# widdowquinn/pyani

Hardware: AMD Instinct MI355X
Metric: genome-pairs/sec (ordered pairs) + wall-clock for the N x N ANIm grid: nucmer --mum + delta-filter -1 + parse_delta equivalent per ordered pair, genomes resident in HBM; vs the CPU path on this box's host cores (higher is better)
Workload: dtype u32 packed DP words (score << 17 | state << 15 | errors), i64 lengths, f64 identity

## Files before the change

### include/pyani_gpu.h

```cpp
#ifndef PYANI_GPU_H
#define PYANI_GPU_H

#include <stdint.h>

#ifdef __cplusplus
extern "C" {
#endif

#define PG_OK 0
#define PG_E_ARG (-1)
#define PG_E_NODEVICE (-2)
#define PG_E_HIP (-3)
#define PG_E_IO (-4)
#define PG_E_NOMEM (-5)
#define PG_E_KEYSET (-6)
#define PG_E_EMPTY (-7)
#define PG_E_RNA (-8)
#define PG_E_CAPACITY (-9)
#define PG_E_INTERNAL (-10)

typedef struct pg_ctx pg_ctx;

const char* pg_version(void);
int pg_create(pg_ctx** out, int device);
void pg_destroy(pg_ctx* ctx);
const char* pg_last_error(const pg_ctx* ctx);
int pg_sync(pg_ctx* ctx);

int pg_add_genome(pg_ctx* ctx, const uint8_t* seq, const uint64_t* rec_off, uint32_t n_rec, int32_t* genome_id_out);
int pg_add_fasta(pg_ctx* ctx, const char* path, int32_t* genome_id_out, uint64_t* total_len_out, uint32_t* n_rec_out);
int pg_add_fasta_batch(pg_ctx* ctx, const char* const* paths, uint32_t n, uint32_t threads, int32_t* genome_ids_out,
                       uint64_t* total_len_out, uint32_t* n_rec_out);
int pg_genome_count(const pg_ctx* ctx);
int pg_genome_length(const pg_ctx* ctx, int32_t genome_id, uint64_t* total_len_out, uint32_t* n_rec_out);
int pg_clear_genomes(pg_ctx* ctx);
int pg_upload(pg_ctx* ctx);
int pg_tetra_algorithmic_bytes(const pg_ctx* ctx, const int32_t* genome_ids, uint32_t n, uint64_t* bytes_out,
                               uint64_t* bases_out);

int pg_tetra_counts(pg_ctx* ctx, const int32_t* genome_ids, uint32_t n, uint64_t* c2, uint64_t* c3, uint64_t* c4);

int pg_tetra_zscores(pg_ctx* ctx, const uint64_t* c2, const uint64_t* c3, const uint64_t* c4, uint32_t n, double* z,
                     uint8_t* present);

int pg_tetra_corr(pg_ctx* ctx, const double* z, const uint8_t* present, uint32_t n, double* out);

int pg_tetra_matrix(pg_ctx* ctx, const int32_t* genome_ids, uint32_t n, double* z_out, uint8_t* present_out,
                    double* corr_out);
int pg_tetra_matrix_enqueue(pg_ctx* ctx, const int32_t* genome_ids, uint32_t n, int fetch_z);
int pg_tetra_matrix_fetch(pg_ctx* ctx, uint32_t n, double* z_out, uint8_t* present_out, double* corr_out);

int pg_tetra_zscores_dev(pg_ctx* ctx, const int32_t* genome_ids, uint32_t n, double* d_z, uint8_t* d_present);
int pg_tetra_corr_rows_dev(pg_ctx* ctx, const double* d_z, const uint8_t* d_present, uint32_t n, uint32_t row0,
                           uint32_t nrows, double* d_out);

typedef struct {
  int64_t ref_aln_len, qry_aln_len, sim_errors, n_alignments;
  double identity;
  int32_t status;
  int32_t reserved;
} pg_anim_result;
#define PG_ANIM_NO_ALIGNMENT 1
int pg_anim_pairs(pg_ctx* ctx, const int32_t* ref_ids, const int32_t* qry_ids, uint64_t n_pairs, int maxmatch,
                  int filter_1to1, pg_anim_result* out);
int pg_anim_pairs_enqueue(pg_ctx* ctx, const int32_t* ref_ids, const int32_t* qry_ids, uint64_t n_pairs, int maxmatch,
                          int filter_1to1, uint64_t* ticket);
int pg_anim_pairs_fetch(pg_ctx* ctx, uint64_t ticket, pg_anim_result* out, uint64_t n_pairs);

#define PG_EXTENDER_NUCMER 0
int pg_anim_set_extender(pg_ctx* ctx, int extender);
int pg_anim_set_workers(pg_ctx* ctx, int workers);

int pg_anim_counters(pg_ctx* ctx, uint64_t* out, int reset);

int pg_anim_set_batch_budget(pg_ctx* ctx, uint32_t max_pairs, uint64_t max_matches);

typedef struct {
  int32_t ref_rec, qry_rec;
  int32_t rs, re, qs, qe;
  int32_t errors;
  int32_t kept;
} pg_anim_alignment;
int pg_anim_pair_alignments(pg_ctx* ctx, int32_t ref_id, int32_t qry_id, pg_anim_alignment* out, uint32_t cap, uint32_t* n_out);

int pg_anim_alignments_batch(pg_ctx* ctx, const int32_t* ref_ids, const int32_t* qry_ids, uint64_t n_pairs, int maxmatch, int with_indels,
                             uint64_t* aln_offsets, uint64_t* n_indels);
int pg_anim_alignments_read(pg_ctx* ctx, pg_anim_alignment* out, uint64_t* indel_offsets, int64_t* indels);

int pg_anim_reduce(pg_ctx* ctx, uint32_t n_pairs, const uint64_t* offsets, const int32_t* rseq, const int32_t* qseq,
                   const int32_t* rs, const int32_t* re, const int32_t* qs, const int32_t* qe, const int32_t* errors,
                   int apply_filter, pg_anim_result* out);

int pg_anib_reduce(pg_ctx* ctx, uint32_t n_pairs, const uint64_t* offsets, const uint32_t* n_frags, const int32_t* frag,
                   const int32_t* length, const int32_t* mismatch, const int32_t* gaps, const int32_t* qlen, const double* pident,
                   int64_t* aln_length_out, int64_t* sim_errors_out, double* pid_out);

typedef struct {
  int64_t aln_length, sim_errors;
  double pid;
  int32_t n_frags, n_kept;
  int32_t status, reserved;
} pg_anib_result;
int pg_anib_pairs(pg_ctx* ctx, const int32_t* qry_ids, const int32_t* sbj_ids, uint64_t n_pairs, uint32_t fragsize, pg_anib_result* out);
typedef struct {
  int32_t frag, length, mismatch, gaps, nident, qlen, qstart, qend, sstart, send, srec, score;
} pg_anib_row;
int pg_anib_pair_rows(pg_ctx* ctx, int32_t qry_id, int32_t sbj_id, uint32_t fragsize, pg_anib_row* out, uint32_t cap, uint32_t* n_out);

typedef struct {
  double ani;
  int32_t matches;
  int32_t fragments;
  int32_t status;
  int32_t reserved;
} pg_sketch_result;
#define PG_SKETCH_NO_RESULT 1
int pg_sketch_pairs(pg_ctx* ctx, const int32_t* qry_ids, const int32_t* ref_ids, uint64_t n_pairs, int32_t frag_len, int32_t scale,
                    double min_fraction, pg_sketch_result* out);

int pg_profile_enable(pg_ctx* ctx, int on);
int pg_profile_config(pg_ctx* ctx, uint32_t kernel_mask, uint32_t every_n);
int pg_profile_reset(pg_ctx* ctx);
#define PG_K_TETRA_COUNT 0
#define PG_K_TETRA_FINALIZE 1
#define PG_K_TETRA_STATS 2
#define PG_K_TETRA_PAIRS 3
#define PG_K_ANIM_SEED 4
#define PG_K_ANIM_HIT 5
#define PG_K_ANIM_CLUSTER 6
#define PG_K_ANIM_GAPS 7
#define PG_K_ANIM_EXTLANE 8
#define PG_K_ANIM_EXTEND 9
#define PG_K_ANIM_FINISH 10
#define PG_K_ANIB_BUCKET 11
#define PG_K_ANIB_FRAG 12
#define PG_K_ANIM_FWD 13
#define PG_K_ANIM_BWD 14
#define PG_K_SKETCH_PAIRS 15
#define PG_K__COUNT 16
int pg_profile_get(pg_ctx* ctx, int which, double* total_ms_out, uint64_t* launches_out);
const char* pg_kernel_name(int which);

#ifdef __cplusplus
}
#endif
#endif
```

### pyani_amd/_lib.py

```python
import ctypes
import os
from pathlib import Path



def configure_runtime(hw_queues: int = 2) -> bool:
    if not 1 <= int(hw_queues) <= 2:
        raise ValueError(f"hw_queues must be 1 or 2, not {hw_queues}")
    os.environ.setdefault("GPU_MAX_HW_QUEUES", str(int(hw_queues)))
    return _lib is None

LIB_PATH = Path(__file__).resolve().parent / "libpyani_gpu.so"

PG_OK, PG_E_ARG, PG_E_NODEVICE, PG_E_HIP, PG_E_IO, PG_E_NOMEM, PG_E_KEYSET, PG_E_EMPTY, PG_E_RNA = 0, -1, -2, -3, -4, -5, -6, -7, -8
PG_E_CAPACITY, PG_ANIM_NO_ALIGNMENT = -9, 1
K_TETRA_COUNT, K_TETRA_FINALIZE, K_TETRA_STATS, K_TETRA_PAIRS = 0, 1, 2, 3
(K_ANIM_SEED, K_ANIM_HIT, K_ANIM_CLUSTER, K_ANIM_GAPS, K_ANIM_EXTLANE, K_ANIM_EXTEND, K_ANIM_FINISH) = 4, 5, 6, 7, 8, 9, 10
K_ANIB_BUCKET, K_ANIB_FRAG = 11, 12
K_ANIM_FWD, K_ANIM_BWD = 13, 14
K_SKETCH_PAIRS = 15
K_COUNT = 16
PG_SKETCH_NO_RESULT = 1

_vp, _i32, _u32, _u64, _int = ctypes.c_void_p, ctypes.c_int32, ctypes.c_uint32, ctypes.c_uint64, ctypes.c_int
_P = ctypes.POINTER
SIGNATURES = {
    "pg_version": (ctypes.c_char_p, []),
    "pg_create": (_int, [_P(_vp), _int]),
    "pg_destroy": (None, [_vp]),
    "pg_last_error": (ctypes.c_char_p, [_vp]),
    "pg_sync": (_int, [_vp]),
    "pg_add_genome": (_int, [_vp, _vp, _vp, _u32, _P(_i32)]),
    "pg_add_fasta": (_int, [_vp, ctypes.c_char_p, _P(_i32), _P(_u64), _P(_u32)]),
    "pg_add_fasta_batch": (_int, [_vp, _vp, _u32, _u32, _vp, _vp, _vp]),
    "pg_genome_count": (_int, [_vp]),
    "pg_genome_length": (_int, [_vp, _i32, _P(_u64), _P(_u32)]),
    "pg_clear_genomes": (_int, [_vp]),
    "pg_upload": (_int, [_vp]),
    "pg_tetra_algorithmic_bytes": (_int, [_vp, _vp, _u32, _P(_u64), _P(_u64)]),
    "pg_tetra_counts": (_int, [_vp, _vp, _u32, _vp, _vp, _vp]),
    "pg_tetra_zscores": (_int, [_vp, _vp, _vp, _vp, _u32, _vp, _vp]),
    "pg_tetra_corr": (_int, [_vp, _vp, _vp, _u32, _vp]),
    "pg_tetra_matrix": (_int, [_vp, _vp, _u32, _vp, _vp, _vp]),
    "pg_tetra_matrix_enqueue": (_int, [_vp, _vp, _u32, _int]),
    "pg_tetra_matrix_fetch": (_int, [_vp, _u32, _vp, _vp, _vp]),
    "pg_tetra_zscores_dev": (_int, [_vp, _vp, _u32, _vp, _vp]),
    "pg_tetra_corr_rows_dev": (_int, [_vp, _vp, _vp, _u32, _u32, _u32, _vp]),
    "pg_anim_pairs": (_int, [_vp, _vp, _vp, _u64, _int, _int, _vp]),
    "pg_anim_pairs_enqueue": (_int, [_vp, _vp, _vp, _u64, _int, _int, _vp]),
    "pg_anim_pairs_fetch": (_int, [_vp, _u64, _vp, _u64]),
    "pg_anim_reduce": (_int, [_vp, _u32, _vp, _vp, _vp, _vp, _vp, _vp, _vp, _vp, _int, _vp]),
    "pg_anim_set_batch_budget": (_int, [_vp, _u32, ctypes.c_uint64]),
    "pg_anim_set_workers": (_int, [_vp, _int]),
    "pg_anim_set_extender": (_int, [_vp, _int]),
    "pg_anim_counters": (_int, [_vp, _vp, _int]),
    "pg_anim_pair_alignments": (_int, [_vp, _i32, _i32, _vp, _u32, _P(_u32)]),
    "pg_anim_alignments_batch": (_int, [_vp, _vp, _vp, _u64, _int, _int, _vp, _P(_u64)]),
    "pg_anim_alignments_read": (_int, [_vp, _vp, _vp, _vp]),
    "pg_anib_reduce": (_int, [_vp, _u32, _vp, _vp, _vp, _vp, _vp, _vp, _vp, _vp, _vp, _vp, _vp]),
    "pg_anib_pairs": (_int, [_vp, _vp, _vp, _u64, _u32, _vp]),
    "pg_anib_pair_rows": (_int, [_vp, _i32, _i32, _u32, _vp, _u32, _P(_u32)]),
    "pg_sketch_pairs": (_int, [_vp, _vp, _vp, _u64, _i32, _i32, ctypes.c_double, _vp]),
    "pg_profile_enable": (_int, [_vp, _int]),
    "pg_profile_config": (_int, [_vp, _u32, _u32]),
    "pg_profile_reset": (_int, [_vp]),
    "pg_profile_get": (_int, [_vp, _int, _P(ctypes.c_double), _P(_u64)]),
    "pg_kernel_name": (ctypes.c_char_p, [_int]),
}

_lib = None


class PyaniGpuError(RuntimeError):

    def __init__(self, code, msg):
        super().__init__(f"libpyani_gpu error {code}: {msg}")
        self.code = code


def load():
    global _lib
    if _lib is None:
        if not LIB_PATH.exists():
            raise ImportError(f"{LIB_PATH} not built — run `python -m pyani_amd.build` (needs hipcc); "
                              "pyani_amd has no CPU fallback")
        lib = ctypes.CDLL(str(LIB_PATH))
        for name, (res, args) in SIGNATURES.items():
            fn = getattr(lib, name)
            fn.restype, fn.argtypes = res, args
        _lib = lib
    return _lib
```

### pyani_amd/csrc/pg_anim.hip

```cpp
#include <tuple>
#include "pg_internal.h"
#include "pg_anim_core.h"
#include "pg_nucmer_core.h"
#include "pg_nucmer_diag.h"
#include "pg_anib_core.h"
#include "pg_anim_trace.h"

using namespace pga;

namespace {

constexpr unsigned long long SLOT_EMPTY = ~0ull;
constexpr int FRAG_SEED_MIN = 16;

struct RefDesc {
  const uint32_t* codes;
  const uint32_t* mask;
  int32_t len;
  const int32_t* rec_start;
  int32_t n_rec;
};

struct UnitDesc {
  const uint32_t* codes;
// ... 70 lines not shown
  int32_t *nch = nullptr, *status = nullptr;
  pg_anim_result* out = nullptr;
  Match *mem = nullptr, *cm = nullptr;
  int32_t *iscratch = nullptr, *order = nullptr;
  Chain* chains = nullptr;
  FinishScratch S{};
  uint2* wl_d = nullptr;
  Match* seedbuf = nullptr;
  size_t seed_cap = 0;
  uint32_t* seed_total = nullptr;
  Match* hits_d = nullptr;
  Match* hits_sorted = nullptr;
  uint32_t *hit_count = nullptr, *hoff = nullptr, *hit_cursor = nullptr;
  size_t hit_cap = 0;
  int32_t* mirror_d = nullptr;
  BigUnit* big_d = nullptr;
  uint2* ranges_d = nullptr;
  RangeOut* range_out = nullptr;
  size_t big_cap = 0, range_cap = 0;
  bool lds_attr_set = false;
  pgn::PnAln* pn = nullptr;
  uint8_t* pn_fused = nullptr;
  int32_t* pn_n = nullptr;
  uint32_t* pn_cursor = nullptr;
  uint32_t* pn_gscratch = nullptr;
  uint32_t* pn_wide = nullptr;
  PnForcedReq* pn_reqs = nullptr;
  pgn::PnGap* pn_gaps = nullptr;
  pgn::PnFwd* pn_fwd = nullptr;
  pgn::PnBwd* pn_bwd = nullptr;
  pgn::PnTurn* pn_tlog = nullptr;
  int32_t* pn_born = nullptr;
  uint32_t* pn_porder = nullptr;
  pgn::PnPiece* pn_pieces = nullptr;
  uint32_t* pn_npieces = nullptr;
  size_t pn_piece_cap = 0, pn_npieces_cap = 0;
  uint8_t* tr_arena = nullptr;
  uint32_t* tr_out = nullptr;
  PnTraceJob* tr_jobs = nullptr;
  unsigned long long *tr_off = nullptr, *tr_cursor = nullptr;
  int32_t* tr_cnt = nullptr;
  size_t tr_arena_cap = 0, tr_out_cap = 0, tr_jobs_cap = 0;
  PnGapTask* pn_tasks = nullptr;
  uint32_t* pn_order = nullptr;
  size_t pn_cap = 0, pn_units = 0, pn_waves = 0, pn_req_cap = 0, pn_req_n = 0;
  int32_t* fr_tables = nullptr;
  FragPair* fr_pairs = nullptr;
  uint32_t *fr_slot_pair = nullptr, *fr_off = nullptr, *fr_nrows = nullptr;
  uint64_t* fr_ebase = nullptr;
  FragSeed* fr_entries = nullptr;
  FragRow* fr_rows = nullptr;
  pg_anib_result* fr_out = nullptr;
  uint32_t *fr_list = nullptr, *fr_nlist = nullptr, *fr_wtmp = nullptr;
  WordIdx* fr_widx = nullptr;
  size_t fr_list_cap = 0, fr_widx_cap = 0;
  size_t fr_tables_cap = 0, fr_pairs_cap = 0, fr_slots_cap = 0, fr_off_cap = 0, fr_units_cap = 0, fr_entries_cap = 0;
};

template <typename T>
int regrow(pg_ctx* ctx, T*& p, size_t n) {
  if (p) PG_HIP(ctx, hipFree(p));
  p = nullptr;
  PG_HIP(ctx, hipMalloc(reinterpret_cast<void**>(&p), (n ? n : 1) * sizeof(T)));
  return PG_OK;
}
}

static AnimScratch* anim_scratch(pg_ctx* ctx) {
  void*& slot = tls_worker ? ctx->anim_scratch_w[tls_worker] : ctx->anim_scratch;
  if (!slot) slot = new AnimScratch();
  return static_cast<AnimScratch*>(slot);
}
static AnimLists* anim_lists(pg_ctx* ctx) {
  if (!ctx->anim_lists) ctx->anim_lists = new AnimLists();
  return static_cast<AnimLists*>(ctx->anim_lists);
}
static hipStream_t cur_stream(pg_ctx* ctx) { return tls_worker ? ctx->stream_w[tls_worker] : ctx->stream; }
void pg_anim_set_worker(pg_ctx* ctx, int worker) {
  tls_worker = worker > 0 && worker < pg_ctx::MAX_WORKERS ? worker : 0;
  pg_tls_stream = cur_stream(ctx);
}

void pg_anim_set_sink(PgAlnSink* sink) { tls_sink = sink; }
int pg_anim_counters_read(pg_ctx* ctx, uint64_t* out, int reset) {
  PG_HIP(ctx, hipDeviceSynchronize());
  unsigned long long a[32], b[32], z[32] = {0};
  PG_HIP(ctx, hipMemcpyFromSymbol(a, HIP_SYMBOL(g_pn_stats), sizeof(a)));
  PG_HIP(ctx, hipMemcpyFromSymbol(b, HIP_SYMBOL(g_pn_kstats), sizeof(b)));
  for (int i = 0; i < 32; ++i) { out[i] = a[i]; out[32 + i] = b[i]; }
  if (reset) {
    PG_HIP(ctx, hipMemcpyToSymbol(HIP_SYMBOL(g_pn_stats), z, sizeof(z)));
    PG_HIP(ctx, hipMemcpyToSymbol(HIP_SYMBOL(g_pn_kstats), z, sizeof(z)));
  }
  return PG_OK;
}

void pg_anim_drop_lists(pg_ctx* ctx) {
  std::lock_guard<std::mutex> lk(ctx->anim_mu);
  AnimLists* A = static_cast<AnimLists*>(ctx->anim_lists);
  if (!A) return;
  for (auto& g : A->gidx) {
    void* ptrs[] = {g.ref_list, g.qry_list, g.ref_goff, g.qry_goff, g.qry_list1, g.qry_goff1, g.word_start, g.word_pos};
    for (void* p : ptrs) if (p) (void)hipFree(p);
  }
  A->gidx.clear();
}

static int anim_ensure_lists(pg_ctx* ctx, AnimScratch* A, const std::vector<int32_t>& ref_genomes, const std::vector<int32_t>& qry_genomes,
                             int qstep) {
  std::lock_guard<std::mutex> lk(ctx->anim_mu);
  AnimLists* LS = anim_lists(ctx);
  if (LS->gidx.size() < ctx->genomes.size()) LS->gidx.resize(ctx->genomes.size());
  std::vector<std::pair<uint64_t**, uint32_t**>> mine;
  const int rc_all = [&]() -> int {
  int rc;
  bool built = false;
  if (!A->list_cnt && (rc = regrow(ctx, A->list_cnt, (size_t)2 * SEED_GROUPS))) return rc;
  std::vector<int32_t> fresh_refs;
  for (int role = 0; role < 2; ++role) {
    for (int32_t gid : role ? qry_genomes : ref_genomes) {
      GenomeIdx& X = LS->gidx[gid];
      uint64_t*& qlist = qstep == 1 ? X.qry_list1 : X.qry_list;
      uint32_t*& qgoff = qstep == 1 ? X.qry_goff1 : X.qry_goff;
      if (role ? qlist != nullptr : X.ref_list != nullptr) continue;
      const PgGenome& G = ctx->genomes[gid];
      const int32_t len = (int32_t)G.stream_len;
      const uint32_t n_sub = role ? 2 * SEED_GROUPS : SEED_GROUPS;
      const size_t bound = role ? 2 * ((size_t)len / qstep + 1) : (size_t)len + 1;
      uint64_t*& list = role ? qlist : X.ref_list;
      uint32_t*& goff = role ? qgoff : X.ref_goff;
      mine.emplace_back(&list, &goff);
      if ((rc = regrow(ctx, list, bound))) return rc;
      if ((rc = regrow(ctx, goff, (size_t)n_sub + 2))) return rc;
      const uint32_t* codes = ctx->d_codes + G.arena_start / 16;
      const uint32_t* mask = ctx->d_mask + G.arena_start / 32;
      const int32_t n_idx = role ? len / qstep + 1 : len;
      const dim3 grid((uint32_t)(n_idx + LIST_CHUNK - 1) / LIST_CHUNK, role ? 2 : 1);
      PG_HIP(ctx, hipMemsetAsync(A->list_cnt, 0, (size_t)n_sub * 4, cur_stream(ctx)));
      if (grid.x)
        hipLaunchKernelGGL(anim_list_kernel, grid, dim3(LIST_BLOCK), 0, cur_stream(ctx), codes, mask, len, role, A->list_cnt,
                           (const uint32_t*)nullptr, (uint64_t*)nullptr, 0, qstep);
      hipLaunchKernelGGL(anim_list_scan_kernel, dim3(1), dim3(64), 0, cur_stream(ctx), A->list_cnt, goff, n_sub);
      if (grid.x)
        hipLaunchKernelGGL(anim_list_kernel, grid, dim3(LIST_BLOCK), 0, cur_stream(ctx), codes, mask, len, role, A->list_cnt,
                           (const uint32_t*)goff, list, 1, qstep);
      if (!role) fresh_refs.push_back(gid);
      built = true;
    }
  }
  PG_HIP(ctx, hipGetLastError());
  if (built) PG_HIP(ctx, hipStreamSynchronize(cur_stream(ctx)));
  for (int32_t gid : fresh_refs)
    PG_HIP(ctx, hipMemcpy(&LS->gidx[gid].ref_max, LS->gidx[gid].ref_goff + SEED_GROUPS + 1, 4, hipMemcpyDeviceToHost));
  return PG_OK;
  }();
  if (rc_all != PG_OK) {
    (void)hipStreamSynchronize(cur_stream(ctx));
    for (auto& pr : mine) {
      if (*pr.first) { (void)hipFree(*pr.first); *pr.first = nullptr; }
      if (*pr.second) { (void)hipFree(*pr.second); *pr.second = nullptr; }
    }
  }
  return rc_all;
}

static void anim_free_one(pg_ctx* ctx, void*& slot);
// ... 549 lines not shown
      std::vector<uint32_t> uorder(n_units);
      for (uint32_t u = 0; u < n_units; ++u) uorder[u] = u;
      std::stable_sort(uorder.begin(), uorder.end(), [&](uint32_t a, uint32_t b) { return nch[a] > nch[b]; });
      PG_HIP(ctx, hipMemcpyAsync(A->pn_order, uorder.data(), (size_t)n_units * 4, hipMemcpyHostToDevice, cur_stream(ctx)));
      std::vector<uint32_t> porder(n_pairs);
      for (uint32_t p = 0; p < n_pairs; ++p) porder[p] = p;
      std::stable_sort(porder.begin(), porder.end(), [&](uint32_t a, uint32_t b) { return std::max(nch[2 * a], nch[2 * a + 1]) > std::max(nch[2 * b], nch[2 * b + 1]); });
      PG_HIP(ctx, hipMemcpyAsync(A->pn_porder, porder.data(), (size_t)n_pairs * 4, hipMemcpyHostToDevice, cur_stream(ctx)));
      PG_HIP(ctx, hipStreamSynchronize(cur_stream(ctx)));
    }
    if (!A->pn_cursor && (rc = regrow(ctx, A->pn_cursor, 24))) return rc;
    const uint32_t pn_waves = (uint32_t)ctx->num_cu * 12u;
    const uint32_t pn_walk_waves = (uint32_t)ctx->num_cu * 8u;
    const uint32_t pn_waves_pre = (uint32_t)ctx->num_cu * 32u;
    const uint32_t pn_waves_scr = ctx->anim_gap_lanes ? (pn_waves > pn_walk_waves ? pn_waves : pn_walk_waves) : pn_waves_pre;
    if (pn_waves_scr > A->pn_waves) { if ((rc = regrow(ctx, A->pn_gscratch, (size_t)pn_waves_scr * PN_GLOBAL_WORDS))) return rc; A->pn_waves = pn_waves_scr; }
    const bool trace = tls_sink && tls_sink->with_indels;
    const bool bwd_ahead = ctx->anim_bwd_ahead != 0;
    if (trace) {
      const size_t need = pn_piece_base(Mp, (uint32_t)n_wl, n_units) + 16;
      if (need > A->pn_piece_cap) { if ((rc = regrow(ctx, A->pn_pieces, need))) return rc; A->pn_piece_cap = need; }
      if (n_units > A->pn_npieces_cap) { if ((rc = regrow(ctx, A->pn_npieces, (size_t)n_units + 16))) return rc; A->pn_npieces_cap = (size_t)n_units + 16; }
      PG_HIP(ctx, hipMemsetAsync(A->pn_npieces, 0, (size_t)n_units * 4, cur_stream(ctx)));
    }
    const size_t req_cap = Mp + 16;
    A->pn_req_n = req_cap;
    if (req_cap > A->pn_req_cap) { if ((rc = regrow(ctx, A->pn_reqs, req_cap + req_cap / 2))) return rc; if ((rc = regrow(ctx, A->pn_wide, 3 * (req_cap + req_cap / 2)))) return rc; A->pn_req_cap = req_cap + req_cap / 2; }
    PG_HIP(ctx, hipMemsetAsync(A->pn_cursor, 0, 96, cur_stream(ctx)));
    if (n_wl && trace) PG_HIP(ctx, hipMemcpyAsync(A->choff_d, choff.data(), choff.size() * 4, hipMemcpyHostToDevice, cur_stream(ctx)));
    if (n_wl && !trace) {
      if (n_wl > A->wl) { if ((rc = regrow(ctx, A->wl_d, n_wl + n_wl / 2))) return rc; A->wl = n_wl + n_wl / 2; }
      PG_HIP(ctx, hipMemcpyAsync(A->choff_d, choff.data(), choff.size() * 4, hipMemcpyHostToDevice, cur_stream(ctx)));
      hipLaunchKernelGGL(anim_wl_kernel, dim3(n_units), dim3(64), 0, cur_stream(ctx), A->choff_d, A->wl_d);
      pg_prof_begin(ctx, PG_K_ANIM_GAPS);
      const int lane_small = ctx->anim_gap_lanes;
      if (lane_small) {
        hipLaunchKernelGGL(anim_postnuc_gaplist_kernel, dim3((uint32_t)((n_wl + 255) / 256)), dim3(256), 0, cur_stream(ctx), A->units_d, O, A->wl_d,
                           (uint32_t)n_wl, A->pn_tasks, A->pn_cap, A->pn_cursor + 4);
        const dim3 lg((uint32_t)ctx->num_cu * 8u);
        hipLaunchKernelGGL((anim_postnuc_gaplane_kernel<16>), lg, dim3(64), 0, cur_stream(ctx), A->refs_d, A->units_d, O, A->pn_tasks, A->pn_cursor + 4, A->pn_gaps);
        hipLaunchKernelGGL((anim_postnuc_gaplane_kernel<32>), lg, dim3(64), 0, cur_stream(ctx), A->refs_d, A->units_d, O, A->pn_tasks + A->pn_cap, A->pn_cursor + 5, A->pn_gaps);
        hipLaunchKernelGGL((anim_postnuc_gaplane_kernel<PN_SMALL>), lg, dim3(64), 0, cur_stream(ctx), A->refs_d, A->units_d, O, A->pn_tasks + 2 * A->pn_cap, A->pn_cursor + 6, A->pn_gaps);
      }
      if (lane_small)
        hipLaunchKernelGGL(anim_postnuc_gapbig_kernel, dim3(pn_waves_pre), dim3(64), 0, cur_stream(ctx), A->refs_d, A->units_d, O, A->pn_cursor + 3,
                           A->pn_gaps, A->pn_tasks + 3 * A->pn_cap, A->pn_cursor + 11);
      else
        hipLaunchKernelGGL(anim_postnuc_gap_kernel, dim3(pn_waves_pre), dim3(64), 0, cur_stream(ctx), A->refs_d, A->units_d, O, A->wl_d, (uint32_t)n_wl,
                           A->pn_cursor + 3, A->pn_gaps, A->pn_gscratch);
      pg_prof_end(ctx);
      pg_prof_begin(ctx, PG_K_ANIM_FWD);
      hipLaunchKernelGGL(anim_postnuc_fwd_kernel, dim3(pn_waves_pre), dim3(64), 0, cur_stream(ctx), A->refs_d, A->units_d, O, A->wl_d, (uint32_t)n_wl,
                         A->pn_cursor + 8, A->pn_fwd, A->pn_gscratch);
      pg_prof_end(ctx);
      pg_prof_begin(ctx, PG_K_ANIM_BWD);
      if (bwd_ahead) {
        PG_HIP(ctx, hipMemsetAsync(A->pn_bwd, 0, (size_t)M * sizeof(pgn::PnBwd), cur_stream(ctx)));
        hipLaunchKernelGGL(anim_postnuc_rehearse_kernel, dim3(pn_walk_waves < n_units ? pn_walk_waves : n_units), dim3(64), 0, cur_stream(ctx), A->refs_d,
                           A->units_d, n_units, O, A->pn_cursor + 9, A->pn, A->pn_fused, A->pn_gscratch, A->pn_gaps, A->pn_fwd, A->pn_order, A->pn_bwd);
        hipLaunchKernelGGL(anim_postnuc_bwd_kernel, dim3(pn_waves_pre), dim3(64), 0, cur_stream(ctx), A->refs_d, A->units_d, O, A->wl_d, (uint32_t)n_wl,
                           A->pn_cursor + 10, A->pn_bwd, A->pn_gscratch);
      }
      pg_prof_end(ctx);
    }
    pg_prof_begin(ctx, PG_K_ANIM_EXTEND);
    if (n_wl)
      hipLaunchKernelGGL(anim_postnuc_kernel, dim3(pn_walk_waves / 2 < n_pairs ? pn_walk_waves / 2 : n_pairs), dim3(128), 0, cur_stream(ctx), A->refs_d, A->units_d,
                         n_pairs, O, A->pn_cursor, A->pn, A->pn_fused, A->pn_n, A->pn_gscratch, A->pn_reqs, A->pn_cursor + 1, (uint32_t)req_cap,
                         trace ? nullptr : A->pn_gaps, trace ? nullptr : A->pn_fwd, A->pn_porder, trace ? A->pn_pieces : nullptr, A->pn_npieces, A->choff_d,
                         bwd_ahead && !trace ? A->pn_bwd : nullptr, A->pn_tlog, A->pn_born);
    else
      PG_HIP(ctx, hipMemsetAsync(A->pn_n, 0, (size_t)n_units * 4, cur_stream(ctx)));
    pg_prof_end(ctx);
    pg_prof_begin(ctx, PG_K_ANIM_EXTLANE);
    if (n_wl) {
      const uint32_t win_max = (uint32_t)ctx->anim_pn_window_max, group_max = (uint32_t)ctx->anim_pn_group_max;
      hipLaunchKernelGGL(anim_postnuc_forced_kernel, dim3(pn_waves_pre), dim3(64), 0, cur_stream(ctx), A->refs_d, A->units_d, A->pn_reqs,
                         A->pn_cursor + 1, (uint32_t)req_cap, A->pn_cursor + 2, A->pn_n, A->pn_wide, A->pn_cursor + 12, win_max);
      hipLaunchKernelGGL(anim_postnuc_forced_wide_kernel, dim3(pn_waves), dim3(64), 0, cur_stream(ctx), A->refs_d, A->units_d, A->pn_reqs,
                         A->pn_cursor + 1, (uint32_t)req_cap, A->pn_cursor + 13, A->pn_n, A->pn_gscratch, A->pn_wide, A->pn_cursor + 12,
                         A->pn_wide + req_cap, A->pn_cursor + 14, win_max);
      hipLaunchKernelGGL(anim_postnuc_forced_huge_kernel, dim3((uint32_t)ctx->num_cu * 2u), dim3(64 * PN_HUGE_WAVES), 0, cur_stream(ctx), A->refs_d,
                         A->units_d, A->pn_reqs, A->pn_cursor + 15, A->pn_n, A->pn_wide + req_cap, A->pn_cursor + 14, A->pn_wide + 2 * req_cap,
                         A->pn_cursor + 16, group_max);
      hipLaunchKernelGGL(anim_postnuc_forced_strips_kernel, dim3(pn_waves), dim3(64), 0, cur_stream(ctx), A->refs_d, A->units_d, A->pn_reqs,
                         A->pn_cursor + 17, A->pn_n, A->pn_gscratch, A->pn_wide + 2 * req_cap, A->pn_cursor + 16);
    }
    pg_prof_end(ctx);
    if (pg_dev_env("PYANI_PN_STATS")) {
      PG_HIP(ctx, hipStreamSynchronize(cur_stream(ctx)));
      unsigned long long st[32], zero[32] = {0};
      PG_HIP(ctx, hipMemcpyFromSymbol(st, HIP_SYMBOL(g_pn_stats), sizeof(st)));
      PG_HIP(ctx, hipMemcpyToSymbol(HIP_SYMBOL(g_pn_stats), zero, sizeof(zero)));
      fprintf(stderr, "[pn-stats] units %llu clusters %llu | regs: calls %llu steps %llu cells %llu moves %llu overflows %llu | lds: calls %llu steps %llu cells %llu | "
                      "global: calls %llu steps %llu cells %llu\n", st[11], st[12], st[0], st[1], st[2], st[9], st[10], st[3], st[4], st[5], st[6], st[7], st[8]);
      fprintf(stderr, "[pn-stats] searches of the gap + units kernels: %llu calls, %.1f ms inside the engine (summed over waves); shadow tests that asked for the synteny's current alignment: %llu\n", st[22], st[21] / 1e5, st[31]);
      fprintf(stderr, "[pn-stats] forced passes by engine (127 / 255 / 511 cells / strips): %llu %llu %llu %llu passes, %.1f %.1f %.1f %.1f ms summed over waves\n",
              st[27], st[28], st[29], st[30], st[23] / 1e5, st[24] / 1e5, st[25] / 1e5, st[26] / 1e5);
      {
        unsigned long long ks[32], kz[32] = {0};
        PG_HIP(ctx, hipMemcpyFromSymbol(ks, HIP_SYMBOL(g_pn_kstats), sizeof(ks)));
        PG_HIP(ctx, hipMemcpyToSymbol(HIP_SYMBOL(g_pn_kstats), kz, sizeof(kz)));
        const char* kn[8] = {"gaps", "forward", "backward-ahead", "walks", "forced narrow", "forced 512-1024", "forced 2048", "forced group 8192"};
        for (int k = 0; k < 8; ++k)
          fprintf(stderr, "[pn-stats] diagonal engine in %-16s: %llu calls, %llu anti-diagonals, %llu cells\n", kn[k], ks[4 * k], ks[4 * k + 1], ks[4 * k + 2]);
        fprintf(stderr, "[pn-stats] walk kernel scans: shadow test %.1f ms over %llu rows of 64 alignments, reverse-target search %.1f ms in %llu calls (summed over waves)\n",
                ks[3] / 1e5, ks[7], ks[11] / 1e5, ks[15]);
        fprintf(stderr, "[pn-stats] run-ahead results the walk took: forward %llu of %llu computed (%.4f), backward %llu found ready of %llu searches run ahead; %llu searches left to the walk itself\n",
                ks[19], ks[4], ks[4] ? (double)ks[19] / (double)ks[4] : 0.0, ks[23], ks[8], ks[12]);
      }
      for (int k = 13; k <= 17; k += 4)
        fprintf(stderr, "[pn-stats] %s: busy %.1f ms summed over waves, span %.1f ms, longest item %.1f ms (size %llu)\n", k == 13 ? "units" : "forced",
                st[k] / 1e5, st[k + 2] ? (st[k + 2] - ~st[k + 3]) / 1e5 : 0.0, (st[k + 1] >> 20) / 1e5, st[k + 1] & 0xFFFFFull);
    }
  }
  pg_prof_begin(ctx, PG_K_ANIM_FINISH);
  hipLaunchKernelGGL(anim_finish_kernel, dim3(n_pairs), dim3(64), 0, cur_stream(ctx), A->refs_d, A->units_d, n_pairs,
                     O, A->pn, A->pn_n, A->S, filter_1to1, A->out);
  pg_prof_end(ctx);
  PG_HIP(ctx, hipGetLastError());
  PG_HIP(ctx, hipMemcpyAsync(out_host, A->out, n_pairs * sizeof(pg_anim_result), hipMemcpyDeviceToHost, cur_stream(ctx)));
  PG_HIP(ctx, hipStreamSynchronize(cur_stream(ctx)));
  if (tls_sink && (rc = anim_collect(ctx, A, ref_ids, qry_ids, n_pairs, out_host, choff, *tls_sink))) return rc;
  return PG_OK;
}

static int anib_ensure_word_index(pg_ctx* ctx, AnimScratch* A, int32_t gid) {
  int rc;
  std::lock_guard<std::mutex> lk(ctx->anim_mu);
  AnimLists* LS = anim_lists(ctx);
  if (LS->gidx.size() < ctx->genomes.size()) LS->gidx.resize(ctx->genomes.size());
  GenomeIdx& X = LS->gidx[gid];
  if (X.word_start) return PG_OK;
  const PgGenome& G = ctx->genomes[gid];
  const int32_t len = (int32_t)G.stream_len;
  const uint32_t* codes = ctx->d_codes + G.arena_start / 16;
  const uint32_t* mask = ctx->d_mask + G.arena_start / 32;
  uint32_t* start = nullptr;
  int32_t* pos = nullptr;
  if (!A->fr_wtmp && (rc = regrow(ctx, A->fr_wtmp, (size_t)WORD_BUCKETS + 1024 + 16))) return rc;
  if ((rc = regrow(ctx, start, (size_t)WORD_BUCKETS + 1))) return rc;
  if ((rc = regrow(ctx, pos, (size_t)(len > 0 ? len : 1)))) { (void)hipFree(start); return rc; }
  hipStream_t st = cur_stream(ctx);
  const uint32_t grid = (uint32_t)((len + 255) / 256);
  hipError_t e = hipMemsetAsync(start, 0, ((size_t)WORD_BUCKETS + 1) * 4, st);
  if (e == hipSuccess && grid) hipLaunchKernelGGL(anib_word_count_kernel, dim3(grid), dim3(256), 0, st, codes, mask, len, start, pos, 0);
  if (e == hipSuccess) {
    hipLaunchKernelGGL(anib_word_scan1_kernel, dim3(WORD_BUCKETS / 4096u), dim3(1024), 0, st, start, A->fr_wtmp + WORD_BUCKETS);
    hipLaunchKernelGGL(anib_word_scan2_kernel, dim3(1), dim3(1024), 0, st, A->fr_wtmp + WORD_BUCKETS, WORD_BUCKETS / 4096u, start + WORD_BUCKETS);
    hipLaunchKernelGGL(anib_word_scan3_kernel, dim3(WORD_BUCKETS / 1024u), dim3(1024), 0, st, start, A->fr_wtmp + WORD_BUCKETS, A->fr_wtmp);
    if (grid) hipLaunchKernelGGL(anib_word_count_kernel, dim3(grid), dim3(256), 0, st, codes, mask, len, A->fr_wtmp, pos, 1);
    e = hipGetLastError();
  }
  if (e == hipSuccess) e = hipStreamSynchronize(st);
  if (e != hipSuccess) { (void)hipFree(start); (void)hipFree(pos); return pg_fail(ctx, PG_E_HIP, hipGetErrorString(e)); }
  X.word_start = start; X.word_pos = pos;
  return PG_OK;
}

static int anib_frag_stage(pg_ctx* ctx, AnimScratch* A, const int32_t* qry_ids, uint32_t n_pairs, const std::vector<uint32_t>& cnt,
                           const PgFragArgs& F, const std::vector<int32_t>& ref_list, const std::vector<uint32_t>& ref_of_pair) {
  int rc;
  const uint32_t n_units = 2 * n_pairs;
  std::vector<int32_t> tables;
  struct Tab { size_t pos, len, rec0; int32_t n_frags; };
  std::vector<Tab> tab_of(ctx->genomes.size(), Tab{0, 0, 0, -1});
  std::vector<FragPair> fp(n_pairs);
  std::vector<size_t> tab_ref(n_pairs);
  uint64_t slots = 0;
  for (uint32_t p = 0; p < n_pairs; ++p) {
    const int32_t gid = qry_ids[p];
    Tab& T = tab_of[gid];
    if (T.n_frags < 0) {
      const PgGenome& Q = ctx->genomes[gid];
      std::vector<int32_t> pos, len, rec0;
      for (uint32_t r = 0; r < Q.n_rec; ++r) {
        rec0.push_back((int32_t)pos.size());
        const int32_t r0 = Q.rec_start[r], r1 = Q.rec_start[r + 1] - 1;
        for (int32_t f0 = r0; f0 < r1; f0 += F.fragsize) { pos.push_back(f0); len.push_back(r1 - f0 < F.fragsize ? r1 - f0 : F.fragsize); }
      }
      T.n_frags = (int32_t)pos.size();
      T.pos = tables.size(); tables.insert(tables.end(), pos.begin(), pos.end());
      T.len = tables.size(); tables.insert(tables.end(), len.begin(), len.end());
      T.rec0 = tables.size(); tables.insert(tables.end(), rec0.begin(), rec0.end());
    }
    fp[p].n_frags = T.n_frags;
    fp[p].slot0 = (uint32_t)slots;
    slots += (uint64_t)T.n_frags;
// ... 234 lines not shown
```

### pyani_amd/csrc/pg_api.cpp

```cpp
#include <algorithm>
#include <cstdio>
#include <cstring>
#include <atomic>
#include <functional>
#include <new>
#include <thread>

#include "pg_internal.h"

int pg_fail(pg_ctx* ctx, int code, const std::string& msg) {
  if (ctx) { std::lock_guard<std::mutex> lk(ctx->err_mu); ctx->err = msg; }
  return code;
}

static const char* const KERNEL_NAMES[PG_K__COUNT] = {"tetra_count_kernel", "tetra_finalize_kernel", "tetra_stats_kernel",
                                                      "tetra_pairs_kernel", "anim_seed_kernel", "anim_hit_kernels",
                                                      "anim_cluster_wave_kernel",
                                                      "anim_postnuc_gap_kernels", "anim_postnuc_forced_kernels",
                                                      "anim_postnuc_kernel", "anim_finish_kernel", "anib_bucket_kernel",
                                                      "anib_frag_kernel", "anim_postnuc_fwd_kernel", "anim_postnuc_rehearse_kernel+anim_postnuc_bwd_kernel",
                                                      "sketch_pairs_kernel"};

thread_local hipStream_t pg_tls_stream = nullptr;
namespace { thread_local PgEventPair tls_open_pair; thread_local bool tls_open = false; }
// ... 211 lines not shown
    bytes = off_present + (uint64_t)n * 256;
    bytes_corr_only = off_z;
  }
};

int ensure_result(pg_ctx* ctx, uint32_t n, bool corr) {
  const ResultLayout L(n, corr);
  if (L.bytes > ctx->result_cap) {
    const uint64_t cap = std::max<uint64_t>(L.bytes, ctx->result_cap + ctx->result_cap / 2);
    int rc;
    PG_HIP(ctx, hipStreamSynchronize(ctx->stream));
    if ((rc = dev_realloc(ctx, ctx->d_result, cap))) return rc;
    if ((rc = host_realloc(ctx, ctx->h_result, cap))) return rc;
    PG_HIP(ctx, hipMemsetAsync(ctx->d_result, 0, 16, ctx->stream));
    ctx->result_cap = cap;
  }
  ctx->d_flags = reinterpret_cast<int32_t*>(ctx->d_result);
  ctx->d_z = reinterpret_cast<double*>(ctx->d_result + L.off_z);
  ctx->d_corr = reinterpret_cast<double*>(ctx->d_result + L.off_corr);
  ctx->d_present = ctx->d_result + L.off_present;
  return PG_OK;
}

int ensure_batch(pg_ctx* ctx, const int32_t* ids, uint32_t n) {
  int rc;
  for (uint32_t i = 0; i < n; ++i)
    if (ids[i] < 0 || (size_t)ids[i] >= ctx->genomes.size()) return pg_fail(ctx, PG_E_ARG, "genome id out of range");
  if ((rc = pg_upload(ctx))) return rc;
  if ((rc = ensure_batch_scratch(ctx, n))) return rc;
  if (ctx->batch_ids.size() == n && std::equal(ids, ids + n, ctx->batch_ids.begin()) && n > 0) return PG_OK;
  std::vector<uint32_t> tile0(n), prefix(n + 1, 0), gid(n);
  for (uint32_t b = 0; b < n; ++b) {
    const PgGenome& g = ctx->genomes[ids[b]];
    gid[b] = (uint32_t)ids[b];
    tile0[b] = (uint32_t)(g.arena_start / PG_SUPER);
    prefix[b + 1] = prefix[b] + (uint32_t)(g.padded_len / PG_SUPER);
  }
  ctx->n_work = prefix[n];
  if (n) {
    PG_HIP(ctx, hipMemcpyAsync(ctx->d_seg_tile0, tile0.data(), n * 4, hipMemcpyHostToDevice, ctx->stream));
    PG_HIP(ctx, hipMemcpyAsync(ctx->d_batch_gid, gid.data(), n * 4, hipMemcpyHostToDevice, ctx->stream));
  }
  PG_HIP(ctx, hipMemcpyAsync(ctx->d_seg_prefix, prefix.data(), (n + 1) * 4, hipMemcpyHostToDevice, ctx->stream));
  PG_HIP(ctx, hipStreamSynchronize(ctx->stream));
  ctx->batch_ids.assign(ids, ids + n);
  return PG_OK;
}

int check_flags(pg_ctx* ctx, uint32_t n) {
  const int32_t* h_flags = reinterpret_cast<const int32_t*>(ctx->h_result);
  if (n >= 2) {
    if (h_flags[0] & 1) return pg_fail(ctx, PG_E_KEYSET, "genomes have different observed-tetranucleotide key sets");
    if (h_flags[1] == 0) return pg_fail(ctx, PG_E_EMPTY, "no tetranucleotide observed in any genome");
  }
  return PG_OK;
}

}

extern "C" {

const char* pg_version(void) { return "pyani_gpu 0.1.0 (gfx950)"; }

const char* pg_kernel_name(int which) { return (which >= 0 && which < PG_K__COUNT) ? KERNEL_NAMES[which] : ""; }

int pg_create(pg_ctx** out, int device) {
  if (!out) return PG_E_ARG;
  *out = nullptr;
  int ndev = 0;
  if (hipGetDeviceCount(&ndev) != hipSuccess || ndev <= 0) return PG_E_NODEVICE;
  if (device < 0 || device >= ndev) return PG_E_ARG;
  pg_ctx* ctx = new (std::nothrow) pg_ctx();
  if (!ctx) return PG_E_NOMEM;
  ctx->device = device;
  if (hipSetDevice(device) != hipSuccess || hipStreamCreateWithFlags(&ctx->stream, hipStreamNonBlocking) != hipSuccess) {
    delete ctx;
    return PG_E_HIP;
  }
  for (int w = 1; w < pg_ctx::MAX_WORKERS; ++w)
    if (hipStreamCreateWithFlags(&ctx->stream_w[w], hipStreamNonBlocking) != hipSuccess) { delete ctx; return PG_E_HIP; }
  if (const char* g = pg_dev_env("PYANI_ANIM_BWD_AHEAD")) ctx->anim_bwd_ahead = atoi(g) != 0;
  if (const char* g = pg_dev_env("PYANI_PN_WINDOW_MAX")) ctx->anim_pn_window_max = atoi(g);
  if (const char* g = pg_dev_env("PYANI_PN_GROUP_MAX")) ctx->anim_pn_group_max = atoi(g);
  if (const char* g = pg_dev_env("PYANI_ANIM_GAP_LANES")) ctx->anim_gap_lanes = atoi(g) != 0;
  if (const char* w = pg_dev_env("PYANI_ANIM_WORKERS")) {
    ctx->anim_workers = atoi(w);
    if (ctx->anim_workers < 1) ctx->anim_workers = 1;
    if (ctx->anim_workers > pg_ctx::MAX_WORKERS) ctx->anim_workers = pg_ctx::MAX_WORKERS;
  }
  hipDeviceProp_t prop;
  if (hipGetDeviceProperties(&prop, device) == hipSuccess && prop.multiProcessorCount > 0)
    ctx->num_cu = prop.multiProcessorCount;
  (void)hipGetLastError();
  *out = ctx;
  return PG_OK;
}

void pg_destroy(pg_ctx* ctx) {
  if (!ctx) return;
  for (auto& J : ctx->anim_async) if (J.th.joinable()) J.th.join();
  (void)hipSetDevice(ctx->device);
  (void)hipStreamSynchronize(ctx->stream);
  for (int w = 1; w < pg_ctx::MAX_WORKERS; ++w) (void)hipStreamSynchronize(ctx->stream_w[w]);
  pg_anim_free_scratch(ctx);
  pg_sketch_drop(ctx);
  prof_drain(ctx);
  void* dev[] = {ctx->d_codes, ctx->d_mask, ctx->d_quirk, ctx->d_seg_tile0, ctx->d_seg_prefix, ctx->d_batch_gid, ctx->d_acc,
                 ctx->d_counts, ctx->d_z, ctx->d_present, ctx->d_dev, ctx->d_ss, ctx->d_flags, ctx->d_corr};
  for (void* p : dev)
    if (p) (void)hipFree(p);
  void* host[] = {ctx->h_result, ctx->h_counts};
  for (void* p : host)
    if (p) (void)hipHostFree(p);
  (void)hipStreamDestroy(ctx->stream);
  for (int w = 1; w < pg_ctx::MAX_WORKERS; ++w) (void)hipStreamDestroy(ctx->stream_w[w]);
  (void)hipGetLastError();
  delete ctx;
}

const char* pg_last_error(const pg_ctx* ctx) { return ctx ? ctx->err.c_str() : "null context"; }

int pg_sync(pg_ctx* ctx) {
  if (!ctx) return PG_E_ARG;
  PG_HIP(ctx, hipSetDevice(ctx->device));
  PG_HIP(ctx, hipStreamSynchronize(ctx->stream));
  for (int w = 1; w < pg_ctx::MAX_WORKERS; ++w) PG_HIP(ctx, hipStreamSynchronize(ctx->stream_w[w]));
  return PG_OK;
}

int pg_add_genome(pg_ctx* ctx, const uint8_t* seq, const uint64_t* rec_off, uint32_t n_rec, int32_t* genome_id_out) {
  if (!ctx || !rec_off || (!seq && n_rec && rec_off[n_rec] > rec_off[0])) return pg_fail(ctx, PG_E_ARG, "bad argument");
  for (uint32_t r = 0; r < n_rec; ++r)
    if (rec_off[r + 1] < rec_off[r]) return pg_fail(ctx, PG_E_ARG, "record offsets must be non-decreasing");
  PgGenome g;
  const int rc = pack_genome(seq, rec_off, n_rec, g);
  if (rc == PG_E_RNA)
    return pg_fail(ctx, PG_E_RNA, "sequence contains U/u (RNA); Biopython complements it asymmetrically, unsupported");
  return add_packed(ctx, std::move(g), genome_id_out);
}

int pg_add_fasta(pg_ctx* ctx, const char* path, int32_t* genome_id_out, uint64_t* total_len_out, uint32_t* n_rec_out) {
  if (!ctx || !path) return pg_fail(ctx, PG_E_ARG, "bad argument");
  std::vector<uint8_t> txt, seq;
  std::vector<uint64_t> off;
  if (read_file(path, txt) != 0) return pg_fail(ctx, PG_E_IO, std::string("cannot read ") + path);
  parse_fasta(txt, seq, off);
  const uint64_t zero_off[1] = {0};
  const uint32_t n_rec = off.empty() ? 0 : (uint32_t)off.size() - 1;
  PgGenome g;
  const int rc = pack_genome(seq.data(), off.empty() ? zero_off : off.data(), n_rec, g);
  if (rc == PG_E_RNA) return pg_fail(ctx, PG_E_RNA, std::string(path) + ": sequence contains U/u (RNA), unsupported");
  if (total_len_out) *total_len_out = g.total_len;
  if (n_rec_out) *n_rec_out = n_rec;
  return add_packed(ctx, std::move(g), genome_id_out);
}

int pg_add_fasta_batch(pg_ctx* ctx, const char* const* paths, uint32_t n, uint32_t threads, int32_t* genome_ids_out,
                       uint64_t* total_len_out, uint32_t* n_rec_out) {
  if (!ctx || (n && !paths)) return pg_fail(ctx, PG_E_ARG, "bad argument");
  for (uint32_t i = 0; i < n; ++i) if (!paths[i]) return pg_fail(ctx, PG_E_ARG, "bad argument");
  if (threads == 0) threads = std::thread::hardware_concurrency();
  if (threads == 0) threads = 1;
  if (threads > n) threads = n ? n : 1;
  std::vector<PgGenome> packed(n);
  std::vector<int> status(n, PG_OK);
  std::vector<uint32_t> nrec(n, 0);
// ... 258 lines not shown
  if ((rc = ensure_batch_scratch(ctx, n))) return rc;
  if ((rc = ensure_result(ctx, 1, false))) return rc;
  if (n == 0) return PG_OK;
  ctx->batch_ids.clear();
  if ((rc = pg_launch_tetra_stats(ctx, d_z, d_present, n))) return rc;
  if ((rc = pg_launch_tetra_pairs(ctx, n, row0, nrows, d_out, false))) return rc;
  if ((rc = fetch_result_async(ctx, 16))) return rc;
  PG_HIP(ctx, hipStreamSynchronize(ctx->stream));
  return check_flags(ctx, n);
}

static int anim_run_chunks(pg_ctx* ctx, const std::vector<std::pair<uint64_t, uint64_t>>& chunks,
                           const std::function<int(uint64_t, uint64_t, int)>& run, int slot_base = 0, int max_workers = 0) {
  const int cap_w = max_workers > 0 ? max_workers : ctx->anim_workers;
  const int workers = (int)std::min<size_t>((size_t)cap_w, chunks.size() ? chunks.size() : 1);
  std::atomic<size_t> next{0};
  std::atomic<int> first_rc{PG_OK};
  auto body = [&](int w) {
    (void)hipSetDevice(ctx->device);
    pg_anim_set_worker(ctx, slot_base + w);
    for (size_t c; (c = next++) < chunks.size() && first_rc.load() == PG_OK;) {
      int rc;
      try { rc = run(chunks[c].first, chunks[c].second, w); }
      catch (const std::bad_alloc&) { rc = pg_fail(ctx, PG_E_NOMEM, "out of host memory in an ANIm worker"); }
      catch (const std::exception& e) { rc = pg_fail(ctx, PG_E_HIP, std::string("ANIm worker: ") + e.what()); }
      int expect = PG_OK;
      if (rc != PG_OK) first_rc.compare_exchange_strong(expect, rc);
    }
    pg_anim_set_worker(ctx, 0);
    pg_tls_stream = nullptr;
  };
  std::vector<std::thread> others;
  for (int w = 1; w < workers; ++w) others.emplace_back(body, w);
  body(0);
  for (auto& th : others) th.join();
  return first_rc.load();
}

static std::vector<std::pair<uint64_t, uint64_t>> anim_chunks(const int32_t* table_ids, const std::vector<uint64_t>& order, uint64_t max_pairs,
                                                              uint32_t max_refs) {
  std::vector<std::pair<uint64_t, uint64_t>> chunks;
  const uint64_t n = order.size();
  uint64_t i = 0;
  while (i < n) {
    uint64_t j = i;
    uint32_t nrefs = 0;
    int32_t last = -1;
    while (j < n && j - i < max_pairs) {
      const int32_t rid = table_ids[order[j]];
      if (rid != last) { if (nrefs == max_refs) break; ++nrefs; last = rid; }
      ++j;
    }
    chunks.push_back({i, j});
    i = j;
  }
  return chunks;
}

static uint64_t anim_match_budget(pg_ctx* ctx) {
  size_t free_b = 0, total_b = 0;
  if (hipMemGetInfo(&free_b, &total_b) != hipSuccess) { (void)hipGetLastError(); return ctx->anim_batch_matches; }
  const uint64_t fit = (uint64_t)(0.7 * (double)free_b) / 384u;
  const uint64_t floor_ = 4ull << 20;
  return std::max<uint64_t>(floor_, std::min<uint64_t>(ctx->anim_batch_matches, fit + __atomic_load_n(&ctx->anim_scratch_matches_held, __ATOMIC_RELAXED)));
}

int pg_anim_set_batch_budget(pg_ctx* ctx, uint32_t max_pairs, uint64_t max_matches) {
  if (!ctx || max_pairs == 0 || max_matches < 1024) return pg_fail(ctx, PG_E_ARG, "bad argument");
  ctx->anim_batch_pairs = max_pairs;
  ctx->anim_batch_matches = max_matches;
  return PG_OK;
}

int pg_anim_set_extender(pg_ctx* ctx, int extender) {
  if (!ctx) return PG_E_ARG;
  if (extender != PG_EXTENDER_NUCMER) return pg_fail(ctx, PG_E_ARG, "pg_anim_set_extender: only PG_EXTENDER_NUCMER exists (the approximate banded64 extender was retired)");
  return PG_OK;
}

int pg_anim_set_workers(pg_ctx* ctx, int workers) {
  if (!ctx || workers < 1 || workers > pg_ctx::MAX_WORKERS) return pg_fail(ctx, PG_E_ARG, "workers must be 1 ... 4");
  ctx->anim_workers = workers;
  return PG_OK;
}

int pg_anim_counters(pg_ctx* ctx, uint64_t* out, int reset) {
  if (!ctx || !out) return pg_fail(ctx, PG_E_ARG, "bad argument");
  PG_HIP(ctx, hipSetDevice(ctx->device));
  return pg_anim_counters_read(ctx, out, reset);
}

static int anim_pairs_body(pg_ctx* ctx, const int32_t* ref_ids, const int32_t* qry_ids, uint64_t n_pairs, int maxmatch,
                           int filter_1to1, pg_anim_result* out, int slot_base, int lane_workers, int budget_div);

int pg_anim_pairs(pg_ctx* ctx, const int32_t* ref_ids, const int32_t* qry_ids, uint64_t n_pairs, int maxmatch,
                  int filter_1to1, pg_anim_result* out) {
  if (ctx) {
    std::lock_guard<std::mutex> lk(ctx->anim_async_mu);
    if (ctx->anim_async[0].busy || ctx->anim_async[1].busy) return pg_fail(ctx, PG_E_ARG, "pg_anim_pairs while enqueued calls are in flight: fetch them first");
  }
  return anim_pairs_body(ctx, ref_ids, qry_ids, n_pairs, maxmatch, filter_1to1, out, 0, 0, 1);
}

int pg_anim_pairs_enqueue(pg_ctx* ctx, const int32_t* ref_ids, const int32_t* qry_ids, uint64_t n_pairs, int maxmatch,
                          int filter_1to1, uint64_t* ticket) {
  if (!ctx || !ticket || (n_pairs && (!ref_ids || !qry_ids))) return pg_fail(ctx, PG_E_ARG, "bad argument");
  int rc;
  if ((rc = pg_upload(ctx))) return rc;
  std::lock_guard<std::mutex> lk(ctx->anim_async_mu);
  int lane = -1;
  for (int l = 0; l < 2; ++l) if (!ctx->anim_async[l].busy) { lane = l; break; }
  if (lane < 0) return pg_fail(ctx, PG_E_CAPACITY, "two enqueued ANIm calls are in flight: fetch one first");
  if (!ctx->anim_async[0].busy && !ctx->anim_async[1].busy) {
    size_t free_b = 0, total_b = 0;
    (void)hipSetDevice(ctx->device);
    if (hipMemGetInfo(&free_b, &total_b) == hipSuccess && (double)free_b < 0.4 * (double)total_b) pg_anim_release_worker_scratch(ctx);
    (void)hipGetLastError();
  }
  pg_ctx::AnimAsync& J = ctx->anim_async[lane];
  J.r.assign(ref_ids, ref_ids + n_pairs);
  J.q.assign(qry_ids, qry_ids + n_pairs);
  J.out.assign(n_pairs, pg_anim_result{});
  J.ticket = ctx->anim_next_ticket++;
  J.rc = PG_OK;
  J.busy = true;
  const int lane_workers = std::min(2, std::max(1, ctx->anim_workers));
  J.th = std::thread([ctx, &J, lane, lane_workers, maxmatch, filter_1to1]() {
    (void)hipSetDevice(ctx->device);
    try { J.rc = anim_pairs_body(ctx, J.r.data(), J.q.data(), J.r.size(), maxmatch, filter_1to1, J.out.data(), 2 * lane, lane_workers, 2); }
    catch (const std::bad_alloc&) { J.rc = pg_fail(ctx, PG_E_NOMEM, "out of host memory in an enqueued ANIm call"); }
    catch (const std::exception& e) { J.rc = pg_fail(ctx, PG_E_HIP, std::string("enqueued ANIm call: ") + e.what()); }
  });
  *ticket = J.ticket;
  return PG_OK;
}

int pg_anim_pairs_fetch(pg_ctx* ctx, uint64_t ticket, pg_anim_result* out, uint64_t n_pairs) {
  if (!ctx || (n_pairs && !out)) return pg_fail(ctx, PG_E_ARG, "bad argument");
  pg_ctx::AnimAsync* J = nullptr;
  {
    std::lock_guard<std::mutex> lk(ctx->anim_async_mu);
    for (int l = 0; l < 2; ++l) if (ctx->anim_async[l].busy && ctx->anim_async[l].ticket == ticket) J = &ctx->anim_async[l];
  }
  if (!J) return pg_fail(ctx, PG_E_ARG, "no enqueued ANIm call has this ticket");
  if (J->th.joinable()) J->th.join();
  int rc = J->rc;
  if (rc == PG_OK && n_pairs != J->out.size()) rc = pg_fail(ctx, PG_E_ARG, "pg_anim_pairs_fetch: n_pairs differs from the enqueued call's");
  if (rc == PG_OK && n_pairs) memcpy(out, J->out.data(), n_pairs * sizeof(pg_anim_result));
  std::lock_guard<std::mutex> lk(ctx->anim_async_mu);
  J->r.clear(); J->q.clear(); J->out.clear(); J->out.shrink_to_fit();
  J->busy = false;
  return rc;
}

static int anim_pairs_body(pg_ctx* ctx, const int32_t* ref_ids, const int32_t* qry_ids, uint64_t n_pairs, int maxmatch,
                           int filter_1to1, pg_anim_result* out, int slot_base, int lane_workers, int budget_div) {
  if (!ctx || (n_pairs && (!ref_ids || !qry_ids || !out))) return pg_fail(ctx, PG_E_ARG, "bad argument");
  PG_HIP(ctx, hipSetDevice(ctx->device));
  for (uint64_t i = 0; i < n_pairs; ++i)
    if (ref_ids[i] < 0 || (size_t)ref_ids[i] >= ctx->genomes.size() || qry_ids[i] < 0 ||
        (size_t)qry_ids[i] >= ctx->genomes.size())
      return pg_fail(ctx, PG_E_ARG, "genome id out of range");
  int rc;
  if ((rc = pg_upload(ctx))) return rc;
  std::vector<uint64_t> order(n_pairs);
  std::vector<int32_t> hub(n_pairs);
// ... 290 lines not shown
```

### pyani_amd/csrc/pg_internal.h

```cpp
#pragma once
#include <hip/hip_runtime.h>
#include <array>
#include <cstdint>
#include <cstdlib>
#include <mutex>
#include <thread>
#include <string>
#include <vector>

#include "pyani_gpu.h"

constexpr uint32_t PG_SUPER = 65536;
constexpr uint32_t PG_ACC_WORDS = 16 + 64 + 256;

struct PgGenome {
  uint64_t total_len = 0;
  uint32_t n_rec = 0;
  uint64_t stream_len = 0;
  uint64_t padded_len = 0;
  uint64_t arena_start = 0;
  bool resident = false;
  std::vector<uint32_t> codes, mask;
  std::array<uint32_t, 256> quirk{};
  std::vector<int32_t> rec_start;
};

struct PgEventPair {
  hipEvent_t a, b;
  int which;
};

struct pg_ctx {
  int device = 0;
  hipStream_t stream = nullptr;
  std::string err;
  std::mutex mu;
  std::vector<PgGenome> genomes;
  uint64_t arena_used = 0;
  uint32_t* d_codes = nullptr;
  uint32_t* d_mask = nullptr;
  uint64_t arena_cap = 0;
  uint32_t* d_quirk = nullptr;
  uint32_t quirk_cap = 0;
  uint32_t n_resident = 0;
  std::vector<int32_t> batch_ids;
  uint32_t* d_seg_tile0 = nullptr;
  uint32_t* d_seg_prefix = nullptr;
  uint32_t* d_batch_gid = nullptr;
  uint32_t n_work = 0, batch_cap = 0;
  unsigned long long* d_acc = nullptr;
  unsigned long long* d_counts = nullptr;
  double* d_dev = nullptr;
  double* d_ss = nullptr;
  unsigned long long* d_keybits = nullptr;
  uint8_t* d_result = nullptr;
  uint8_t* h_result = nullptr;
  uint64_t result_cap = 0;
  int32_t* d_flags = nullptr;
  double* d_z = nullptr;
  double* d_corr = nullptr;
  uint8_t* d_present = nullptr;
  unsigned long long* h_counts = nullptr;
  uint32_t h_batch_cap = 0;
  bool profiling = false;
  uint32_t prof_mask = 0xFFFFFFFFu, prof_every = 1;
  uint64_t prof_seen[PG_K__COUNT] = {};
  bool prof_open = false;
  std::vector<PgEventPair> events;
  double prof_ms[PG_K__COUNT] = {};
  uint64_t prof_n[PG_K__COUNT] = {};
  int num_cu = 256;
  void* anim_scratch = nullptr;
  std::vector<pg_anim_alignment> aln_store;
  std::vector<uint64_t> aln_indel_off;
  std::vector<int64_t> aln_indels;
  static constexpr int MAX_WORKERS = 4;
  void* anim_scratch_w[MAX_WORKERS] = {nullptr, nullptr, nullptr, nullptr};
  hipStream_t stream_w[MAX_WORKERS] = {nullptr, nullptr, nullptr, nullptr};
  void* anim_lists = nullptr;
  void* sketch_store = nullptr;
  std::mutex anim_mu, err_mu, prof_mu;
  int anib_word_tier = 1;
  int anim_pn_window_max = 2048;
  int anim_pn_group_max = 8184;
  int anim_gap_lanes = 1;
  int anim_bwd_ahead = 1;
  int anim_workers = 2;
  struct AnimAsync {
    std::thread th;
    std::vector<int32_t> r, q;
    std::vector<pg_anim_result> out;
    uint64_t ticket = 0;
    int rc = 0;
    bool busy = false;
  } anim_async[2];
  uint64_t anim_next_ticket = 1;
  std::mutex anim_async_mu;
  uint32_t anim_batch_pairs = 131072;
  uint64_t anim_scratch_matches_held = 0;
  uint64_t anim_batch_matches = 512ull << 20;
};

int pg_fail(pg_ctx* ctx, int code, const std::string& msg);
#define PG_HIP(ctx, call)                                                                                     \
  do {                                                                                                        \
    hipError_t _e = (call);                                                                                   \
    if (_e != hipSuccess)                                                                                     \
      return pg_fail((ctx), PG_E_HIP, std::string(#call) + ": " + hipGetErrorString(_e));                     \
  } while (0)

extern thread_local hipStream_t pg_tls_stream;
void pg_prof_begin(pg_ctx* ctx, int which);
void pg_prof_end(pg_ctx* ctx);

int pg_launch_tetra_count(pg_ctx* ctx, uint32_t n_batch);
int pg_launch_tetra_finalize(pg_ctx* ctx, uint32_t n_batch, unsigned long long* d_acc_in);
int pg_launch_tetra_stats(pg_ctx* ctx, const double* d_z, const uint8_t* d_present, uint32_t n);
int pg_launch_tetra_pairs(pg_ctx* ctx, uint32_t n, uint32_t row0, uint32_t nrows, double* d_out, bool mirror);

int pg_anim_reduce_run(pg_ctx* ctx, uint32_t n_pairs, const uint64_t* offsets, const int32_t* rseq, const int32_t* qseq,
                       const int32_t* rs, const int32_t* re, const int32_t* qs, const int32_t* qe, const int32_t* errors,
                       int apply_filter, pg_anim_result* out);
struct PgFragArgs {
  int32_t fragsize;
  pg_anib_result* out;
  pg_anib_row* rows_out;
  uint32_t rows_cap;
  uint32_t* n_rows_out;
  uint64_t max_slots;
};
int pg_anim_run_batch(pg_ctx* ctx, const int32_t* ref_ids, const int32_t* qry_ids, uint32_t n_pairs, int filter_1to1, int maxmatch,
                      uint64_t max_matches, pg_anim_result* out_host, uint32_t* n_done,
                      const PgFragArgs* frag = nullptr);
void pg_anim_set_worker(pg_ctx* ctx, int worker);
void pg_anim_free_scratch(pg_ctx* ctx);
void pg_anim_release_worker_scratch(pg_ctx* ctx);
int pg_anim_fetch_alignments(pg_ctx* ctx, int32_t ref_id, int32_t qry_id, uint32_t n, pg_anim_alignment* out);
inline const char* pg_dev_env(const char* name) {
  const char* on = getenv("PYANI_DEV_KNOBS");
  return on && on[0] == '1' ? getenv(name) : nullptr;
}
constexpr uint32_t PG_FRAG_MAX_FRAGS = 15872;
struct PgAlnSink {
  bool with_indels = false;
  std::vector<pg_anim_alignment> alns;
  std::vector<uint32_t> pair_count;
  std::vector<std::vector<int64_t>> indels;
};
int pg_anim_counters_read(pg_ctx* ctx, uint64_t* out , int reset);
void pg_anim_set_sink(PgAlnSink* sink);
void pg_anim_drop_lists(pg_ctx* ctx);
void pg_sketch_drop(pg_ctx* ctx);
int pg_anib_reduce_run(pg_ctx* ctx, uint32_t n_pairs, const uint64_t* offsets, const uint32_t* n_frags, const int32_t* frag,
                       const int32_t* length, const int32_t* mismatch, const int32_t* gaps, const int32_t* qlen,
                       const double* pident, int64_t* aln_out, int64_t* err_out, double* pid_out);
```

### pyani_amd/csrc/pg_nucmer_diag.h

```cpp
#pragma once
#include <stdint.h>
#include "pg_nucmer_core.h"

namespace pgd {
using namespace pgn;

template <int DPL> struct DiagRegs { uint32_t X[DPL], D[DPL], I[DPL], mw[DPL]; };

PG_HD uint32_t rev16_fields(uint32_t x) {
#if defined(__HIP_DEVICE_COMPILE__)
  x = __brev(x);
#else
  x = ((x >> 1) & 0x55555555u) | ((x & 0x55555555u) << 1);
  x = ((x >> 2) & 0x33333333u) | ((x & 0x33333333u) << 2);
  x = ((x >> 4) & 0x0F0F0F0Fu) | ((x & 0x0F0F0F0Fu) << 4);
  x = ((x >> 8) & 0x00FF00FFu) | ((x & 0x00FF00FFu) << 8);
  x = (x >> 16) | (x << 16);
#endif
  return ((x & 0x55555555u) << 1) | ((x >> 1) & 0x55555555u);
}
PG_HD uint32_t spread16(uint32_t m) {
  m &= 0xFFFFu;
  m = (m | (m << 8)) & 0x00FF00FFu;
  m = (m | (m << 4)) & 0x0F0F0F0Fu;
  m = (m | (m << 2)) & 0x33333333u;
  m = (m | (m << 1)) & 0x55555555u;
  return m;
}

struct DiagRelabel { uint32_t mask, st_insert, st_match; };
template <int DPL, int PAR, bool NORM = false>
PG_HD uint32_t diag_lane_edge(const DiagRegs<DPL>& T) {
  constexpr int32_t RISE = NORM && PAR == 0 ? GOOD_SCORE : 0;
  const uint32_t c = w_gap(PAR == 0 ? T.D[DPL - 1] : T.I[0], CONT_GAP_SCORE - RISE), x = w_gap(PAR == 0 ? T.X[DPL - 1] : T.X[0], OPEN_GAP_SCORE - RISE);
  return c > x ? c : x;
}
template <int DPL, int PAR, bool TRACK, bool NORM = false>
PG_HD void diag_lane_step(DiagRegs<DPL>& T, uint32_t nbM, uint32_t g0, uint32_t glo, uint32_t gspan, const DiagRelabel& rel,
                          uint32_t& key, uint32_t& keyw) {
  key = 0u; keyw = 0u;
  const uint32_t gofs = g0 - glo;
  constexpr int32_t RISE = NORM && PAR == 0 ? GOOD_SCORE : 0;
#if defined(__HIP_DEVICE_COMPILE__)
#pragma unroll
#endif
  for (int s = PAR; s < DPL; s += 2) {
    uint32_t dm, im;
    if (s == 0) dm = nbM;
    else { const uint32_t dc = w_gap(T.D[s - 1], CONT_GAP_SCORE - RISE), dx = w_gap(T.X[s - 1], OPEN_GAP_SCORE - RISE); dm = dc > dx ? dc : dx; }
    if (s == DPL - 1) im = nbM;
    else { const uint32_t ic = w_gap(T.I[s + 1], CONT_GAP_SCORE - RISE), ix = w_gap(T.X[s + 1], OPEN_GAP_SCORE - RISE); im = ic > ix ? ic : ix; }
    const bool in = (uint32_t)(gofs + (uint32_t)s) <= gspan;
    const uint32_t mk = in ? rel.mask : 0u;
    const uint32_t d = dm & mk , i = s == DPL - 1 ? (im & mk) + rel.st_insert : (im & mk) | rel.st_insert;
    const uint32_t m = ((NORM ? w_step_norm(T.X[s], T.mw[s]) : w_step_window(T.X[s], T.mw[s])) & mk) | rel.st_match;
    T.mw[s] <<= 2;
    T.X[s] = w_max3(d, i, m); T.D[s] = d; T.I[s] = i;
    if (TRACK) {
      const uint32_t k = (T.X[s] & ~(W_ONE - 1u)) | (g0 + (uint32_t)s);
      if (k >= key) { key = k; keyw = T.X[s]; }
    }
  }
}
template <int DPL, int PAR>
PG_HD void diag_lane_key(const DiagRegs<DPL>& T, uint32_t g0, uint32_t& key, uint32_t& keyw) {
  key = 0u; keyw = 0u;
#if defined(__HIP_DEVICE_COMPILE__)
#pragma unroll
#endif
  for (int s = PAR; s < DPL; s += 2) {
    const uint32_t k = (T.X[s] & ~(W_ONE - 1u)) | (g0 + (uint32_t)s);
    if (k >= key) { key = k; keyw = T.X[s]; }
  }
}
template <int DPL, int PAR>
PG_HD uint32_t diag_lane_top(const DiagRegs<DPL>& T) {
  uint32_t top = 0u;
#if defined(__HIP_DEVICE_COMPILE__)
#pragma unroll
#endif
  for (int s = PAR; s < DPL; s += 2) top = T.X[s] > top ? T.X[s] : top;
  return top;
}
template <int DPL, int PAR>
PG_HD uint32_t diag_lane_alive(const DiagRegs<DPL>& T, uint32_t thr) {
  uint32_t bits = 0u;
  for (int s = PAR; s < DPL; s += 2) bits |= (T.X[s] >= thr ? 1u : 0u) << s;
  return bits;
}
template <int DPL, int PAR, bool NORM = false, bool CLEAN = false>
PG_HD void diag_lane_refill(DiagRegs<DPL>& T, uint64_t ca, uint32_t oka, uint64_t cb, uint32_t okb) {
  constexpr int e_last = ((DPL - 1) ^ PAR) & 1, e_0 = PAR & 1;
#if defined(__HIP_DEVICE_COMPILE__)
#pragma unroll
#endif
  for (int s = 0; s < DPL; ++s) {
    const int e_s = (s ^ PAR) & 1;
    const int oa = (DPL - 1 - s + e_s - e_last) / 2, ob = (s + e_s - e_0) / 2;
    const uint32_t a16 = (uint32_t)(ca >> (2 * oa)), b16 = (uint32_t)(cb >> (2 * ob));
    const uint32_t x = a16 ^ b16;
    const uint32_t eq = ~(x | (x >> 1)) & 0x55555555u;
    const uint32_t hit = CLEAN ? eq : eq & spread16((oka >> oa) & (okb >> ob));
    T.mw[s] = rev16_fields(NORM ? hit ^ 0x55555555u : hit) << 1;
  }
}
template <int DPL, int PAR>
PG_HD void diag_refill_origin(int32_t Dct, int32_t k0, int32_t& ia0, int32_t& jb0) {
  constexpr int e_last = ((DPL - 1) ^ PAR) & 1, e_0 = PAR & 1;
  const int32_t u = Dct - k0;
  ia0 = (u - (DPL - 1) + e_last) >> 1;
  jb0 = ((u + e_0) >> 1) + k0;
}

struct DiagCtl {
  int32_t N, M, NM;
  bool fwd, forced, optimal, banded;
  int32_t Dct, Dend;
  int32_t ga, gb;
  int32_t lo, hi;
  int32_t c1g, c2g;
  int32_t kming, kmaxg;
  int32_t shiftk;
  uint32_t high_f, high_w;
  uint32_t high_fw, thr_w;
  int32_t FinishCt, FinishG, FinishShift;
  uint32_t span_sum;
  int32_t wmax;
  int32_t next_refill;
  template <int DPL>
  PG_HD void init(int32_t N_, int32_t M_, unsigned m_o, int32_t band_w) {
    constexpr int32_t HALF = 32 * DPL;
    N = N_; M = M_; NM = N_ + M_;
    fwd = m_o & DIRECTION_BIT; forced = m_o & FORCED_BIT; optimal = m_o & OPTIMAL_BIT; banded = band_w >= 0;
    kming = (M - N < 0 ? M - N : 0) - band_w + HALF; kmaxg = (M - N > 0 ? M - N : 0) + band_w + HALF;
    Dct = 1; Dend = forced ? NM : (NM < BREAK_LEN ? NM : BREAK_LEN);
    ga = HALF - 1; gb = HALF + 1; lo = HALF; hi = HALF; shiftk = 0;
    c1g = 1 - 2 * N + HALF; c2g = 2 * M - 1 + HALF;
    high_f = 0u; high_w = 0u; FinishCt = 0; FinishG = HALF; FinishShift = 0;
    high_fw = 0u; thr_w = (0u - (uint32_t)MAX_DIFF) << SCORE_SHIFT;
    span_sum = 0u; wmax = 0; next_refill = 1;
  }
  template <bool FORCED>
  PG_HD int begin_step() {
    if (Dct > Dend) return 1;
    lo = ga > c1g ? ga : c1g; hi = gb < c2g ? gb : c2g;
    if (FORCED && banded) {
      if (lo < kming) lo = kming;
      if (hi > kmaxg) hi = kmaxg;
      if ((lo + Dct) & 1) ++lo;
      if ((hi + Dct) & 1) --hi;
    }
    return lo > hi ? 2 : 0;
  }
  template <bool FORCED>
  PG_HD bool begin_step_go() {
    lo = ga > c1g ? ga : c1g; hi = gb < c2g ? gb : c2g;
    if (FORCED && banded) {
      if (lo < kming) lo = kming;
      if (hi > kmaxg) hi = kmaxg;
      if ((lo + Dct) & 1) ++lo;
      if ((hi + Dct) & 1) --hi;
    }
    return ((Dend - Dct) | (hi - lo)) >= 0;
  }
  template <int DPL>
  PG_HD int32_t window_check() const {
    constexpr int32_t W = 64 * DPL, HALF = W / 2;
    if (lo >= 2 && hi <= W - 3) return 0;
    if (hi - lo + 5 > W) return INT32_MIN;
    int32_t n = ((lo + hi) / 2 - HALF) / DPL;
    if (n == 0) n = lo < 2 ? -1 : 1;
    if (lo - DPL * n < 2 || hi - DPL * n > W - 3) return INT32_MIN;
    return n;
  }
  template <int DPL>
  PG_HD void window_move(int32_t n) { window_shift(DPL * n); }
  PG_HD void window_shift(int32_t d) {
    shiftk += d; lo -= d; hi -= d; ga -= d; gb -= d; c1g -= d; c2g -= d; kming -= d; kmaxg -= d;
    next_refill = Dct;
  }
  template <bool WIDEST>
  PG_HD void note_cells() {
    span_sum += (uint32_t)(hi - lo);
    if (WIDEST) { const int32_t w = (hi - lo) / 2 + 1; if (w > wmax) wmax = w; }
  }
  PG_HD int32_t steps() const { return Dct - 1; }
  PG_HD unsigned long long cells_total() const { return (unsigned long long)(span_sum / 2u) + (unsigned long long)steps(); }
  PG_HD void update_best(uint32_t gk, uint32_t gw) {
    const uint32_t f = gk >> SCORE_SHIFT;
    if (f >= (high_fw >> SCORE_SHIFT)) {
      high_f = f; high_w = gw; high_fw = f << SCORE_SHIFT; thr_w = (f - (uint32_t)MAX_DIFF) << SCORE_SHIFT; FinishCt = Dct; FinishG = (int32_t)(gk & (W_ONE - 1u)); FinishShift = shiftk;
      Dend = Dct + BREAK_LEN < NM ? Dct + BREAK_LEN : NM;
    }
  }
  PG_HD uint32_t trim_threshold() const { return thr_w; }
  template <bool FORCED, bool NORM_EVEN = false>
  PG_HD void end_step(bool any, uint32_t gmin, uint32_t gmax) {
    if (FORCED) { ga = lo - 1; gb = hi + 1; }
    else if (any) { ga = (int32_t)gmin - 1; gb = (int32_t)gmax + 1; }
    else { ga = 0; gb = 1; Dend = -1; }
    ++Dct; ++c1g; --c2g;
    if (NORM_EVEN) { high_fw -= (uint32_t)GOOD_SCORE << SCORE_SHIFT; thr_w -= (uint32_t)GOOD_SCORE << SCORE_SHIFT; }
  }
  template <int DPL>
  PG_HD bool finish1(bool& reached, uint32_t& corner_slot, int32_t& FinishK) {
    constexpr int32_t HALF = 32 * DPL;
    reached = false;
    const int32_t last = Dct - 1;
    corner_slot = 0u;
    FinishK = FinishG - HALF + FinishShift;
    if (last == NM) {
      if (!optimal) { reached = true; FinishCt = NM; FinishK = M - N; corner_slot = (uint32_t)(M - N - shiftk + HALF); return true; }
      if (FinishCt == last) reached = true;
    }
    return false;
  }
  template <bool NORM = false>
  PG_HD void finish2(uint32_t fin_w, int32_t FinishK, int32_t Astart, int32_t Bstart, int32_t& Aend, int32_t& Bend, int32_t& errors, int32_t& score) const {
    const int32_t fi = (FinishCt - FinishK) / 2, fj = (FinishCt + FinishK) / 2;
    Aend = fwd ? Astart + fi - 1 : Astart - fi + 1;
    Bend = fwd ? Bstart + fj - 1 : Bstart - fj + 1;
    errors = (int32_t)w_errors(fin_w);
    score = NORM ? (int32_t)(fin_w >> SCORE_SHIFT) - (int32_t)NORM_BIAS + norm_offset(FinishCt) : w_score(fin_w);
  }
};

#if !defined(__HIP_DEVICE_COMPILE__)
template <int DPL, typename RefT, typename QryT>
struct DiagWaveEmu {
  static constexpr int W = 64 * DPL, HALF = W / 2;
  const RefT& R;
  const QryT& Q;
  long cells = 0, calls = 0, moves = 0, fails = 0;
  uint32_t last_cells = 0, last_wmax = 0;
  DiagRegs<DPL> T[64];
  template <int PAR, bool NORM>
  void refill(const DiagCtl& C, int32_t Astart, int32_t Bstart) {
    for (int l = 0; l < 64; ++l) {
      const int32_t k0 = DPL * l - HALF + C.shiftk;
      int32_t ia0, jb0;
      diag_refill_origin<DPL, PAR>(C.Dct, k0, ia0, jb0);
      uint64_t ca = 0, cb = 0; uint32_t oka = 0, okb = 0;
      for (int f = 0; f < 32; ++f) {
        const int64_t pa = C.fwd ? (int64_t)Astart + (ia0 + f) - 1 : (int64_t)Astart - (ia0 + f) + 1;
        const int64_t pb = C.fwd ? (int64_t)Bstart + (jb0 + f) - 1 : (int64_t)Bstart - (jb0 + f) + 1;
        if (R.clean(pa)) { ca |= (uint64_t)R.base(pa) << (2 * f); oka |= 1u << f; }
        if (Q.clean(pb)) { cb |= (uint64_t)Q.base(pb) << (2 * f); okb |= 1u << f; }
      }
      if ((oka & okb) == 0xFFFFFFFFu) diag_lane_refill<DPL, PAR, NORM, true>(T[l], ca, oka, cb, okb);
      else diag_lane_refill<DPL, PAR, NORM, false>(T[l], ca, oka, cb, okb);
    }
  }
  template <int PAR, bool FORCED>
  void step(DiagCtl& C) {
    uint32_t nbM[64], key[64], keyw[64];
    for (int l = 0; l < 64; ++l) {
      if (PAR == 0) nbM[l] = l > 0 ? diag_lane_edge<DPL, PAR, !FORCED>(T[l - 1]) : 0u;
      else nbM[l] = l < 63 ? diag_lane_edge<DPL, PAR, !FORCED>(T[l + 1]) : 0u;
    }
    for (int l = 0; l < 64; ++l)
      diag_lane_step<DPL, PAR, !FORCED, !FORCED>(T[l], nbM[l], (uint32_t)(DPL * l), (uint32_t)C.lo, (uint32_t)(C.hi - C.lo), DiagRelabel{~W_STATE, ST_INSERT, ST_MATCH}, key[l], keyw[l]);
    bool any = false; uint32_t gmin = 0, gmax = 0;
    if (!FORCED) {
      uint32_t gk = 0, gw = 0;
      for (int l = 0; l < 64; ++l) if (key[l] > gk) { gk = key[l]; gw = keyw[l]; }
      C.update_best(gk, gw);
      const uint32_t thr = C.trim_threshold();
      for (int l = 0; l < 64; ++l) {
        const uint32_t bits = diag_lane_alive<DPL, PAR>(T[l], thr);
        for (int s = PAR; s < DPL; s += 2)
          if ((bits >> s) & 1u) { const uint32_t g = (uint32_t)(DPL * l + s); if (!any) { gmin = g; any = true; } gmax = g; }
      }
    }
    C.template end_step<FORCED, !FORCED && PAR == 1>(any, gmin, gmax);
  }
  template <bool FORCED>
  bool run_(int32_t Astart, int32_t& Aend, int32_t Bstart, int32_t& Bend, unsigned m_o, int32_t band_w, int32_t& errors, int32_t& score, bool& reached) {
    DiagCtl C;
    const bool fwd = m_o & DIRECTION_BIT;
    C.template init<DPL>(fwd ? Aend - Astart + 1 : Astart - Aend + 1, fwd ? Bend - Bstart + 1 : Bstart - Bend + 1, m_o, band_w);
    for (int l = 0; l < 64; ++l) for (int s = 0; s < DPL; ++s) { T[l].X[s] = 0u; T[l].D[s] = 0u; T[l].I[s] = 0u; T[l].mw[s] = 0u; }
    T[HALF / DPL].X[0] = FORCED ? w_make(0, 0, ST_MATCH) : (NORM_BIAS << SCORE_SHIFT) | ST_MATCH;
    ++calls;
    for (;;) {
      if (C.template begin_step<FORCED>()) break;
      const int32_t n = C.template window_check<DPL>();
      if (n == INT32_MIN) { ++fails; return false; }
      if (n != 0) {
        DiagRegs<DPL> Z;
        for (int s = 0; s < DPL; ++s) { Z.X[s] = 0u; Z.D[s] = 0u; Z.I[s] = 0u; Z.mw[s] = 0u; }
        DiagRegs<DPL> U[64];
        for (int l = 0; l < 64; ++l) U[l] = (l + n >= 0 && l + n < 64) ? T[l + n] : Z;
        for (int l = 0; l < 64; ++l) T[l] = U[l];
        C.template window_move<DPL>(n);
        ++moves;
      }
      if (C.Dct == C.next_refill) { if (C.Dct & 1) refill<1, !FORCED>(C, Astart, Bstart); else refill<0, !FORCED>(C, Astart, Bstart); C.next_refill = C.Dct + 32; }
      C.template note_cells<true>();
      if (C.Dct & 1) step<1, FORCED>(C); else step<0, FORCED>(C);
    }
    uint32_t corner = 0, fin_w = C.high_w;
    int32_t FinishK = 0;
    if (C.template finish1<DPL>(reached, corner, FinishK)) fin_w = T[corner / DPL].X[corner % DPL];
    C.template finish2<!FORCED>(fin_w, FinishK, Astart, Bstart, Aend, Bend, errors, score);
    const unsigned long long nc = C.cells_total();
    cells += (long)nc;
    last_cells = nc > 0xFFFFFFFFull ? 0xFFFFFFFFu : (uint32_t)nc; last_wmax = (uint32_t)C.wmax;
    return true;
  }
  bool run(int32_t Astart, int32_t& Aend, int32_t Bstart, int32_t& Bend, unsigned m_o, int32_t band_w, int32_t& errors, int32_t& score, bool& reached) {
    return (m_o & FORCED_BIT) ? run_<true>(Astart, Aend, Bstart, Bend, m_o, band_w, errors, score, reached)
                              : run_<false>(Astart, Aend, Bstart, Bend, m_o, band_w, errors, score, reached);
  }
};
#endif

PG_HD bool diag_window_holds(int64_t span, int dpl) { return span <= 64 * (int64_t)dpl - 2 * (int64_t)dpl + 2; }
#if !defined(__HIP_DEVICE_COMPILE__)
template <typename RefT, typename QryT>
struct DiagWaveEngine {
  ScalarEngine<RefT, QryT> slow;
  DiagWaveEmu<2, RefT, QryT> e2;
  DiagWaveEmu<4, RefT, QryT> e4;
  DiagWaveEmu<6, RefT, QryT> e6;
  DiagWaveEmu<8, RefT, QryT> e8;
  DiagWaveEmu<12, RefT, QryT> e12;
  DiagWaveEmu<16, RefT, QryT> e16;
  DiagWaveEmu<24, RefT, QryT> e24;
  DiagWaveEmu<32, RefT, QryT> e32;
  long fallbacks = 0;
  void (*fallback_log)(int32_t N, int32_t M, unsigned m_o, int32_t band_w) = nullptr;
  DiagWaveEngine(const RefT& R, const QryT& Q, Cell* d0, Cell* d1, Cell* d2, int32_t cap)
      : slow{R, Q, d0, d1, d2, cap}, e2{R, Q}, e4{R, Q}, e6{R, Q}, e8{R, Q}, e12{R, Q}, e16{R, Q}, e24{R, Q}, e32{R, Q} {}
  bool gap_ready(int32_t, PnGap&) const { return false; }
  void piece(uint32_t, int32_t, int32_t, int32_t, int32_t, int32_t, int32_t, int32_t, unsigned) {}
  bool bwd_ready(int, PnBwd&) const { return false; }
  void bwd_key(int, int32_t, int32_t, int32_t, int32_t, unsigned) {}
  bool fwd_ready(int, PnFwd&) const { return false; }
  int32_t forced_errors(int32_t A0, int32_t A1, int32_t B0, int32_t B1, PnAln*) {
    int32_t err = 0, a = A1, b = B1;
    align(A0, a, B0, b, FORCED_FORWARD_ALIGN, err);
    return err;
  }
  bool shadowed(const Chain* chains, const PnAln* al, int from, int c, int32_t sA, int32_t eA, int32_t sB, int32_t eB) const {
    return PnScalarScans().shadowed(chains, al, from, c, sA, eA, sB, eB); }
  int shadow_first(const Chain* chains, const PnAln* al, int n_al, int c, int32_t sA, int32_t eA, int32_t sB, int32_t eB) const {
    return PnScalarScans().shadow_first(chains, al, n_al, c, sA, eA, sB, eB); }
  int reverse_target(const Chain* chains, const PnAln* al, int cura, int c, int32_t sA, int32_t sB, int32_t dist) const {
    return PnScalarScans().reverse_target(chains, al, cura, c, sA, sB, dist); }
  int forward_target(const Chain* chains, const Match* cm, const int32_t* order, int n, int curk, int c, int32_t sA, int32_t sB,
                     int32_t dist, int32_t& targetA, int32_t& targetB) const {
    return PnScalarScans().forward_target(chains, cm, order, n, curk, c, sA, sB, dist, targetA, targetB); }
  static int window_for(int32_t N, int32_t M, unsigned m_o, int32_t band_w) {
    if (!(m_o & FORCED_BIT)) return 256;
    const int32_t df = N < M ? M - N : N - M;
    const int64_t span = band_w >= 0 ? (int64_t)df + 2 * (int64_t)band_w + 1 : (int64_t)N + M + 1;
    for (int w : {128, 256, 384, 512, 768, 1024, 1536, 2048}) if (diag_window_holds(span + 5, w / 64)) return w;
    return 0;
  }
  bool run(int32_t Astart, int32_t& Aend, int32_t Bstart, int32_t& Bend, unsigned m_o, int32_t band_w, int32_t& errors, int32_t& score) {
    const bool fwd = m_o & DIRECTION_BIT;
    const int32_t N = fwd ? Aend - Astart + 1 : Astart - Aend + 1, M = fwd ? Bend - Bstart + 1 : Bstart - Bend + 1;
    int32_t a = Aend, b = Bend;
    bool reached = false, done = false;
    switch (window_for(N, M, m_o, band_w)) {
      case 128: done = e2.run(Astart, a, Bstart, b, m_o, band_w, errors, score, reached); break;
      case 256: done = e4.run(Astart, a, Bstart, b, m_o, band_w, errors, score, reached); break;
      case 384: done = e6.run(Astart, a, Bstart, b, m_o, band_w, errors, score, reached); break;
      case 512: done = e8.run(Astart, a, Bstart, b, m_o, band_w, errors, score, reached); break;
      case 768: done = e12.run(Astart, a, Bstart, b, m_o, band_w, errors, score, reached); break;
      case 1024: done = e16.run(Astart, a, Bstart, b, m_o, band_w, errors, score, reached); break;
      case 1536: done = e24.run(Astart, a, Bstart, b, m_o, band_w, errors, score, reached); break;
      case 2048: done = e32.run(Astart, a, Bstart, b, m_o, band_w, errors, score, reached); break;
      default: break;
    }
    if (done) { Aend = a; Bend = b; return reached; }
    ++fallbacks;
    if (fallback_log) fallback_log(N, M, m_o, band_w);
    return slow.run(Astart, Aend, Bstart, Bend, m_o, band_w, errors, &score);
  }
  bool align(int32_t Astart, int32_t& Aend, int32_t Bstart, int32_t& Bend, unsigned m_o, int32_t& errors) {
    int32_t score = 0;
    if (!(m_o & FORCED_BIT)) return run(Astart, Aend, Bstart, Bend, m_o, -1, errors, score);
    const bool fwd = m_o & DIRECTION_BIT;
    const int32_t N = fwd ? Aend - Astart + 1 : Astart - Aend + 1, M = fwd ? Bend - Bstart + 1 : Bstart - Bend + 1;
    for (int32_t w = FORCED_BAND_FIRST;;) {
      int32_t a = Aend, b = Bend;
      const bool whole = w >= (N > M ? N : M);
      const bool reached = run(Astart, a, Bstart, b, m_o, whole ? -1 : w, errors, score);
      const int v = slow.overflow ? 0 : forced_verdict(reached, score, whole, N, M, w);
      if (v == 2) { slow.overflow = 1; Aend = a; Bend = b; errors = 0; return false; }
      if (v == 0) { Aend = a; Bend = b; return reached; }
      w = forced_band_after(w, N, M, score);
    }
  }
};
#endif

}
```

### pyani_amd/csrc/pga_postnuc.inc

```

__device__ __forceinline__ void chain_bounds(const RefDesc& R, const UnitDesc& U, const Chain& c, int32_t& r_lo, int32_t& r_hi,
                                             int32_t& q_lo, int32_t& q_hi) {
  r_lo = R.rec_start[c.rrec]; r_hi = R.rec_start[c.rrec + 1] - 1;
  q_lo = U.rec_start[c.qrec]; q_hi = U.rec_start[c.qrec + 1] - 1;
  if (U.strand) { const int32_t a = U.len - q_hi, b = U.len - q_lo; q_lo = a; q_hi = b; }
}
__device__ __forceinline__ uint32_t rev_fields2(uint32_t x) {
  x = __brev(x);
  return ((x & 0x55555555u) << 1) | ((x >> 1) & 0x55555555u);
}
__device__ __forceinline__ uint32_t spread16(uint32_t x) {
  x = (x | (x << 8)) & 0x00FF00FFu;
  x = (x | (x << 4)) & 0x0F0F0F0Fu;
  x = (x | (x << 2)) & 0x33333333u;
  return (x | (x << 1)) & 0x55555555u;
}
__global__ __launch_bounds__(64) void anim_wl_kernel(const uint32_t* __restrict__ choff, uint2* __restrict__ wl) {
  const uint32_t u = blockIdx.x, b = choff[u], n = choff[u + 1] - b;
  for (uint32_t c = threadIdx.x; c < n; c += 64) wl[b + c] = make_uint2(u, c);
}

__device__ unsigned long long g_pn_stats[32];
__device__ unsigned long long g_pn_kstats[32];
__device__ __forceinline__ unsigned long long* pn_stats_lds() { __shared__ unsigned long long s_pn[64]; return s_pn; }
__device__ __forceinline__ void pn_stats_begin() {
  unsigned long long* s = pn_stats_lds();
  s[threadIdx.x & 63] = 0ull;
  __syncthreads();
}
__device__ __forceinline__ void pn_stats_flush() {
  __syncthreads();
  unsigned long long* s = pn_stats_lds();
  const int t = threadIdx.x & 63;
  const unsigned long long v = threadIdx.x < 64 ? s[t] : 0ull;
  if (v) {
    if (t < 32) { if (t == 14 || t == 15 || t == 16 || t == 18 || t == 19 || t == 20) atomicMax(&g_pn_stats[t], v); else atomicAdd(&g_pn_stats[t], v); }
    else atomicAdd(&g_pn_kstats[t - 32], v);
  }
}
__device__ __forceinline__ void pn_stat(int k, unsigned long long v) { if ((threadIdx.x & 63) == 0 && v) atomicAdd(&pn_stats_lds()[k], v); }
__device__ __forceinline__ void pn_stat_max(int k, unsigned long long v) { if ((threadIdx.x & 63) == 0) atomicMax(&pn_stats_lds()[k], v); }
__device__ __forceinline__ void pn_kstat(int k, unsigned long long calls, unsigned long long steps, unsigned long long cells) {
  if ((threadIdx.x & 63) == 0) { unsigned long long* s = pn_stats_lds() + 32 + 4 * k; atomicAdd(&s[0], calls); atomicAdd(&s[1], steps); atomicAdd(&s[2], cells); }
}
__device__ __forceinline__ void pn_stat_item(int k, unsigned long long t0, unsigned long long size) {
  const unsigned long long t1 = wall_clock64(), sz = size < 0xFFFFFull ? size : 0xFFFFFull;
  pn_stat(k, t1 - t0); pn_stat_max(k + 1, ((t1 - t0) << 20) | sz); pn_stat_max(k + 2, t1); pn_stat_max(k + 3, ~t0);
}

constexpr int PN_LDS_CELLS = 256;
constexpr int PN_GLOBAL_CELLS = 16384;
constexpr size_t PN_GLOBAL_WORDS = (size_t)3 * 4 * PN_GLOBAL_CELLS;

template <bool GLOBAL>
struct PnStore {
  static constexpr int CAP = GLOBAL ? PN_GLOBAL_CELLS : PN_LDS_CELLS;
  uint32_t* base;
  __device__ __forceinline__ uint32_t* at(int d, int plane, int32_t j) const { return base + ((d * 4 + plane) * CAP + (j & (CAP - 1))); }
  __device__ __forceinline__ uint32_t ld(int d, int plane, int32_t j) const {
    if (GLOBAL) return __hip_atomic_load(at(d, plane, j), __ATOMIC_RELAXED, __HIP_MEMORY_SCOPE_AGENT);
    return *at(d, plane, j);
  }
  __device__ __forceinline__ void st(int d, int plane, int32_t j, uint32_t v) const {
    if (GLOBAL) __hip_atomic_store(at(d, plane, j), v, __ATOMIC_RELAXED, __HIP_MEMORY_SCOPE_AGENT);
    else *at(d, plane, j) = v;
  }
};

template <bool GLOBAL>
__device__ __forceinline__ void pn_fence() {
  if (GLOBAL) { __builtin_amdgcn_fence(__ATOMIC_SEQ_CST, "agent"); __builtin_amdgcn_wave_barrier(); } else wave_lds_fence();
}

template <bool GLOBAL>
__device__ bool pn_align_wave(const SeqView& R, const StrandView& Q, uint32_t* mem, int32_t Astart, int32_t& Aend, int32_t Bstart,
                              int32_t& Bend, unsigned m_o, int32_t band_w, int32_t& errors, int32_t& score, bool& reached) {
  using namespace pgn;
  const PnStore<GLOBAL> S{mem};
  const int lane = threadIdx.x & 63;
  const bool fwd = m_o & DIRECTION_BIT, forced = m_o & FORCED_BIT;
  const int32_t N = fwd ? Aend - Astart + 1 : Astart - Aend + 1, M = fwd ? Bend - Bstart + 1 : Bstart - Bend + 1;
  int ip2 = 0, ip1 = 1, icur = 2;
  int32_t p2lo = 0, p2hi = -1, p1lo = 0, p1hi = 0;
  pn_fence<GLOBAL>();
  if (lane == 0) { S.st(ip1, 0, 0, 0u); S.st(ip1, 1, 0, 0u); S.st(ip1, 2, 0, w_make(0, 0, ST_MATCH)); S.st(ip1, 3, 0, w_make(0, 0, ST_MATCH)); }
  pn_fence<GLOBAL>();
  int32_t high = -(1 << 30), FinishCt = 0, FinishJ = 0;
  uint32_t high_w = 0;
  int32_t jlo = 0, jhi = 1, Dct;
  bool fits = true;
  unsigned long long stat_cells = 0;
  for (Dct = 1; Dct <= N + M && (forced || Dct - FinishCt <= pgn::BREAK_LEN) && jlo <= jhi; ++Dct) {
    int32_t lo = jlo, hi = jhi;
    if (lo < Dct - N) lo = Dct - N;
    if (lo < 0) lo = 0;
    if (hi > M) hi = M;
    if (hi > Dct) hi = Dct;
    if (band_w >= 0) forced_band_clip(Dct, N, M, band_w, lo, hi);
    if (lo > hi) break;
    if (hi - lo + 1 > PnStore<GLOBAL>::CAP) { fits = false; break; }
    stat_cells += (unsigned long long)(hi - lo + 1);
    uint32_t bestk = 0, bestw = 0;
    for (int32_t c0 = lo; c0 <= hi; c0 += 64) {
      const int32_t j = c0 + lane, i = Dct - j;
      const bool act = j <= hi;
      const bool hasL = act && j >= 1 && j - 1 >= p1lo && j - 1 <= p1hi, hasU = act && i >= 1 && j >= p1lo && j <= p1hi;
      const bool hasG = act && i >= 1 && j >= 1 && j - 1 >= p2lo && j - 1 <= p2hi;
      Cell L{0, 0, 0, 0}, U{0, 0, 0, 0};
      uint32_t G = 0;
      bool sm = false;
      if (hasL) { L.D = S.ld(ip1, 0, j - 1); L.I = S.ld(ip1, 1, j - 1); L.M = S.ld(ip1, 2, j - 1); }
      if (hasU) { U.D = S.ld(ip1, 0, j); U.I = S.ld(ip1, 1, j); U.M = S.ld(ip1, 2, j); }
      if (hasG) {
        G = S.ld(ip2, 3, j - 1);
        const int64_t pa = fwd ? (int64_t)Astart + i - 1 : (int64_t)Astart - i + 1, pb = fwd ? (int64_t)Bstart + j - 1 : (int64_t)Bstart - j + 1;
        sm = R.clean(pa) && Q.clean(pb) && R.base(pa) == Q.base(pb);
      }
      const Cell c = cell_update(L, U, G, sm);
      if (act) {
        S.st(icur, 0, j, c.D); S.st(icur, 1, j, c.I); S.st(icur, 2, j, c.M); S.st(icur, 3, j, c.X);
        const uint32_t key = (c.X & ~(W_ONE - 1u)) | (uint32_t)(j - lo);
        if (key >= bestk) { bestk = key; bestw = c.X; }
      }
    }
    pn_fence<GLOBAL>();
    {
// ... 369 lines not shown
      if (best != 0xFFFFFFFFu) { tgt = t0 - (int)(best & 63u); dist = (int32_t)(best >> 6); }
      if (close) return t0 - stop;
    }
    return tgt;
  }
  __device__ int forward_target(const Chain* chains, const Match* cm, const int32_t* order, int n, int curk, int c, int32_t sA,
                                int32_t sB, int32_t dist, int32_t& targetA, int32_t& targetB) const {
    const int lane = threadIdx.x & 63;
    int targetk = -1;
    const int32_t my_rrec = pn_uni(chains[c].rrec);
    for (int k0 = curk + 1; k0 < n; k0 += 64) {
      if (pn_uni(chains[pn_uni(order[k0])].rrec) > my_rrec) break;
      const int k = k0 + lane;
      pgn::PnCand x{false, false, 0, 0, 0};
      if (k < n) x = pgn::pn_forward_cand(chains, cm, order[k], c, sA, sB);
      const uint64_t close = __ballot(x.valid && x.close);
      const int stop = close ? (int)__builtin_ctzll(close) : 64;
      const uint32_t key = (x.valid && lane < stop && x.dist < dist) ? (((uint32_t)x.dist << 6) | (uint32_t)lane) : 0xFFFFFFFFu;
      const uint32_t best = wave_min_u32(key);
      int pick = -1;
      if (best != 0xFFFFFFFFu) { pick = (int)(best & 63u); dist = (int32_t)(best >> 6); }
      if (close) pick = stop;
      if (pick >= 0) {
        targetk = k0 + pick;
        targetA = __builtin_amdgcn_readlane(x.a, __builtin_amdgcn_readfirstlane(pick));
        targetB = __builtin_amdgcn_readlane(x.b, __builtin_amdgcn_readfirstlane(pick));
      }
      if (close) break;
    }
    return targetk;
  }
  __device__ bool align(int32_t Astart, int32_t& Aend, int32_t Bstart, int32_t& Bend, unsigned m_o, int32_t& errors) {
    int32_t score = 0, a = Aend, b = Bend;
    bool reached = false;
    const unsigned long long t0 = wall_clock64();
    PnRunInfo info{0ull, 0};
    PnRunInfo* const ip = pieces ? &info : nullptr;
    bool in_regs = pn_align_diag<4>(R, Q, Astart, a, Bstart, b, m_o, -1, errors, score, reached, ip, kstat);
    if (DIAG_ONLY) {
      if (!in_regs) { overflow = 1; a = Astart; b = Bstart; errors = 0; reached = false; }
      Aend = a; Bend = b;
      return reached;
    }
    if (!in_regs) { a = Aend; b = Bend; in_regs = pn_align_diag<8>(R, Q, Astart, a, Bstart, b, m_o, -1, errors, score, reached, ip, kstat); }
    last_cells = in_regs && info.cells < 0xFFFFFFFFull ? (uint32_t)info.cells : 0xFFFFFFFFu; last_wmax = (uint32_t)info.wmax;
    pn_stat(21, (unsigned long long)wall_clock64() - t0); pn_stat(22, 1);
    if (in_regs) { Aend = a; Bend = b; return reached; }
    a = Aend; b = Bend;
    if (!pn_align_wave<true>(R, Q, glob, Astart, a, Bstart, b, m_o, -1, errors, score, reached)) { overflow = 1; a = Astart; b = Bstart; errors = 0; reached = false; }
    Aend = a; Bend = b;
    return reached;
  }
  __device__ int32_t forced_errors(int32_t A0, int32_t A1, int32_t B0, int32_t B1, pgn::PnAln* dst) {
    const bool big = (A1 - A0) + (B1 - B0) > 1500;
    uint32_t at = 0;
    if ((threadIdx.x & 63) == 0) at = atomicAdd(big ? n_reqs + 6 : n_reqs, 1u);
    at = (uint32_t)__builtin_amdgcn_readfirstlane((int)at);
    if (at < req_cap) { if ((threadIdx.x & 63) == 0) reqs[big ? req_cap - 1 - at : at] = PnForcedReq{A0, A1, B0, B1, unit, 0, dst}; }
    else overflow = 1;
    last_req = big ? req_cap - 1 - at : at;
    return 0;
  }
};
using PnWaveEngine = PnWaveEngineT<false>;
using PnWaveEngineDiag = PnWaveEngineT<true>;

template <bool WIDE, bool STRIPS = false>
__device__ int pn_forced_wave(const SeqView& R, const StrandView& Q, uint32_t* lds, uint32_t* glob, int32_t A0, int32_t A1, int32_t B0,
                              int32_t B1, int32_t w_start, int32_t& errors, int32_t& w_used, int32_t& w_next, uint32_t win_max = 2048u) {
  const unsigned m_o = pgn::FORCED_FORWARD_ALIGN;
  A0 = pn_uni(A0); A1 = pn_uni(A1); B0 = pn_uni(B0); B1 = pn_uni(B1);
  const int32_t N = A1 - A0 + 1, M = B1 - B0 + 1;
  const int32_t mn = N < M ? N : M, mx = N < M ? M : N;
  int32_t score = 0;
  for (int32_t w = pn_uni(w_start);;) {
    int32_t a = A1, b = B1;
    const bool whole = w >= mx;
    const int32_t widest = whole ? mn + 1 : ((mx - mn + 2 * w) >> 1) + 2, bw = whole ? -1 : w;
    bool reached = false, done = false;
    const int64_t span = (whole ? (int64_t)N + M + 1 : (int64_t)(mx - mn) + 2 * (int64_t)w + 1) + 5;
    if (!WIDE && (!pgd::diag_window_holds(span, 8) || win_max < 128u)) { w_next = w; return 1; }
    const unsigned long long t0 = wall_clock64();
    const int cls = span <= 256 ? 0 : span <= 512 ? 1 : span <= 2048 ? 2 : 3;
#define PN_TRY_DIAG(DPL_, KSTAT_) \
    if (!done && 64u * DPL_ <= win_max && pgd::diag_window_holds(span, DPL_)) { a = A1; b = B1; done = pn_align_diag<DPL_>(R, Q, A0, a, B0, b, m_o, bw, errors, score, reached, nullptr, KSTAT_); }
    if (!WIDE) {
      PN_TRY_DIAG(2, 4) PN_TRY_DIAG(4, 4) PN_TRY_DIAG(6, 4) PN_TRY_DIAG(8, 4)
      if (!done) { w_next = w; return 1; }
    } else {
      PN_TRY_DIAG(8, 5) PN_TRY_DIAG(12, 5) PN_TRY_DIAG(16, 5) PN_TRY_DIAG(24, 6) PN_TRY_DIAG(32, 6)
#undef PN_TRY_DIAG
      if (done) {}
      else if (!STRIPS) { w_next = w; return 1; }
      else if ((size_t)(N + 1) * 8 <= PN_GLOBAL_WORDS) {
        done = true;
        uint32_t* buf[2] = {glob, glob + PN_GLOBAL_WORDS / 2};
        int k = 0;
        for (int32_t j0 = 0; j0 <= M && done; j0 += 511, ++k) {
          const int32_t j1 = j0 + 511 < M + 1 ? j0 + 511 : M + 1;
          const PnStrip st{j0, j1, j0 > 0 ? buf[(k + 1) & 1] : nullptr, j1 < M + 1 ? buf[k & 1] : nullptr};
          a = A1; b = B1;
          __syncthreads();
          done = pn_align_regs<9>(R, Q, A0, a, B0, b, m_o, bw, errors, score, reached, &st);
        }
      }
      if (!done) { a = A1; b = B1; if (widest <= PN_LDS_CELLS) done = pn_align_wave<false>(R, Q, lds, A0, a, B0, b, m_o, bw, errors, score, reached); }
      if (!done) { a = A1; b = B1; done = pn_align_wave<true>(R, Q, glob, A0, a, B0, b, m_o, bw, errors, score, reached); }
    }
    pn_stat(23 + cls, (unsigned long long)wall_clock64() - t0); pn_stat(27 + cls, 1);
    if (!done) { if (!WIDE) { w_next = w; return 1; } return 2; }
    const int v = pgn::forced_verdict(reached, score, whole, N, M, w);
    if (v == 2) return 2;
    if (v == 0) { w_used = bw; return 0; }
    w = pgn::forced_band_after(w, N, M, score);
  }
}

template <bool WIDE>
__device__ __forceinline__ void pn_forced_body(const RefDesc* __restrict__ refs, const UnitDesc* __restrict__ units, PnForcedReq* __restrict__ reqs,
                                               const uint32_t* __restrict__ n_reqs, uint32_t req_cap, uint32_t* __restrict__ cursor,
                                               int32_t* __restrict__ pn_n, uint32_t* __restrict__ gscratch, uint32_t* __restrict__ wide,
                                               uint32_t* __restrict__ n_wide, uint32_t* lds, uint32_t* s_i, uint32_t win_max,
                                               uint32_t* __restrict__ huge = nullptr, uint32_t* __restrict__ n_huge = nullptr) {
  const int lane = threadIdx.x & 63;
  pn_stats_begin();
  const uint32_t n_small = n_reqs[0] < req_cap ? n_reqs[0] : req_cap, n_big = n_reqs[6] < req_cap ? n_reqs[6] : req_cap;
  const uint32_t n_items = WIDE ? *n_wide : n_small + n_big;
  for (;;) {
    __syncthreads();
    if (lane == 0) *s_i = atomicAdd(cursor, 1u);
    __syncthreads();
    const uint32_t i = pn_uni(*s_i);
    if (i >= n_items) break;
    const uint32_t slot = WIDE ? pn_uni(wide[i]) : (i < n_big ? req_cap - 1 - i : i - n_big);
    const PnForcedReq q = reqs[slot];
    const unsigned long long t0 = wall_clock64();
    const UnitDesc U = units[q.unit];
    const RefDesc Rd = refs[U.ref];
    int32_t err = 0, w_used = 0, w_next = 0;
    const int st = pn_forced_wave<WIDE>(SeqView{Rd.codes, Rd.mask, Rd.len}, StrandView{SeqView{U.codes, U.mask, U.len}, U.strand}, lds,
                                        WIDE ? gscratch + (size_t)blockIdx.x * PN_GLOBAL_WORDS : nullptr, q.A0, q.A1, q.B0, q.B1,
                                        WIDE ? q.w : pgn::FORCED_BAND_FIRST, err, w_used, w_next, win_max);
    if (lane == 0) {
      if (st == 1) { reqs[slot].w = w_next; if (WIDE) huge[atomicAdd(n_huge, 1u)] = slot; else wide[atomicAdd(n_wide, 1u)] = slot; }
      else {
        reqs[slot].w = w_used;
        if (st == 2) { const int32_t v = pn_n[q.unit]; if (v >= 0) pn_n[q.unit] = -1 - v; }
        else if (err) atomicAdd(&q.dst->errors, err);
      }
    }
    pn_stat_item(17, t0, (unsigned long long)((q.A1 - q.A0) + (q.B1 - q.B0)));
  }
  pn_stats_flush();
}
__global__ __launch_bounds__(64) void anim_postnuc_forced_kernel(const RefDesc* __restrict__ refs, const UnitDesc* __restrict__ units,
                                                                 PnForcedReq* __restrict__ reqs, const uint32_t* __restrict__ n_reqs,
                                                                 uint32_t req_cap, uint32_t* __restrict__ cursor, int32_t* __restrict__ pn_n,
                                                                 uint32_t* __restrict__ wide, uint32_t* __restrict__ n_wide, uint32_t win_max) {
  __shared__ uint32_t s_i;
  pn_forced_body<false>(refs, units, reqs, n_reqs, req_cap, cursor, pn_n, nullptr, wide, n_wide, nullptr, &s_i, win_max);
}
__global__ __launch_bounds__(64) __attribute__((amdgpu_waves_per_eu(3, 3))) void anim_postnuc_forced_wide_kernel(
    const RefDesc* __restrict__ refs, const UnitDesc* __restrict__ units, PnForcedReq* __restrict__ reqs, const uint32_t* __restrict__ n_reqs,
    uint32_t req_cap, uint32_t* __restrict__ cursor, int32_t* __restrict__ pn_n, uint32_t* __restrict__ gscratch, uint32_t* __restrict__ wide,
    uint32_t* __restrict__ n_wide, uint32_t* __restrict__ huge, uint32_t* __restrict__ n_huge, uint32_t win_max) {
  __shared__ uint32_t lds[3 * 4 * PN_LDS_CELLS];
  __shared__ uint32_t s_i;
  pn_forced_body<true>(refs, units, reqs, n_reqs, req_cap, cursor, pn_n, gscratch, wide, n_wide, lds, &s_i, win_max, huge, n_huge);
}

constexpr int PN_HUGE_WAVES = 4;
__global__ __launch_bounds__(64 * PN_HUGE_WAVES) __attribute__((amdgpu_waves_per_eu(2, 2))) void anim_postnuc_forced_huge_kernel(
    const RefDesc* __restrict__ refs, const UnitDesc* __restrict__ units, PnForcedReq* __restrict__ reqs, uint32_t* __restrict__ cursor,
    int32_t* __restrict__ pn_n, const uint32_t* __restrict__ huge, const uint32_t* __restrict__ n_huge, uint32_t* __restrict__ strips,
    uint32_t* __restrict__ n_strips, uint32_t group_max) {
  __shared__ uint32_t xch[2 * PN_HUGE_WAVES * 4 + 4];
  __shared__ uint32_t s_i;
  const int wave = (int)(threadIdx.x >> 6);
  pn_stats_begin();
  const uint32_t n_items = *n_huge;
  for (;;) {
    __syncthreads();
    if (threadIdx.x == 0) s_i = atomicAdd(cursor, 1u);
    __syncthreads();
    const uint32_t i = pn_uni(s_i);
    if (i >= n_items) break;
    const uint32_t slot = pn_uni(huge[i]);
    const PnForcedReq q = reqs[slot];
    const unsigned long long t0 = wall_clock64();
    const UnitDesc U = units[q.unit];
    const RefDesc Rd = refs[U.ref];
    const SeqView R{Rd.codes, Rd.mask, Rd.len};
    const StrandView Q{SeqView{U.codes, U.mask, U.len}, U.strand};
    const int32_t A0 = pn_uni(q.A0), A1 = pn_uni(q.A1), B0 = pn_uni(q.B0), B1 = pn_uni(q.B1);
    const int32_t N = A1 - A0 + 1, M = B1 - B0 + 1, mn = N < M ? N : M, mx = N < M ? M : N;
    int32_t errors = 0, score = 0, w_used = 0;
    bool handed = false, failed = false;
    for (int32_t w = pn_uni(q.w);;) {
      const bool whole = w >= mx;
      const int32_t bw = whole ? -1 : w;
      const int64_t span = (whole ? (int64_t)N + M + 1 : (int64_t)(mx - mn) + 2 * (int64_t)w + 1) + 5;
      bool done = false;
      const unsigned long long t1 = wall_clock64();
      if (span <= (int64_t)group_max) {
        if (span <= 64 * 12 * PN_HUGE_WAVES - 8) done = pn_forced_diag_group<PN_HUGE_WAVES, 12>(R, Q, A0, A1, B0, B1, bw, xch, errors, score, 7);
        else if (span <= 64 * 16 * PN_HUGE_WAVES - 8) done = pn_forced_diag_group<PN_HUGE_WAVES, 16>(R, Q, A0, A1, B0, B1, bw, xch, errors, score, 7);
        else if (span <= 64 * 24 * PN_HUGE_WAVES - 8) done = pn_forced_diag_group<PN_HUGE_WAVES, 24>(R, Q, A0, A1, B0, B1, bw, xch, errors, score, 7);
        else if (span <= 64 * 32 * PN_HUGE_WAVES - 8) done = pn_forced_diag_group<PN_HUGE_WAVES, 32>(R, Q, A0, A1, B0, B1, bw, xch, errors, score, 7);
      }
      if (!done) {
        if (threadIdx.x == 0) { reqs[slot].w = w; strips[atomicAdd(n_strips, 1u)] = slot; }
        handed = true;
        break;
      }
      if (wave == 0) { pn_stat(26, (unsigned long long)wall_clock64() - t1); pn_stat(30, 1); }
      const int v = pgn::forced_verdict(true, score, whole, N, M, w);
      if (v == 2) { failed = true; break; }
      if (v == 0) { w_used = bw; break; }
      w = pgn::forced_band_after(w, N, M, score);
    }
    if (threadIdx.x == 0 && !handed) {
      reqs[slot].w = w_used;
      if (failed) { const int32_t v = pn_n[q.unit]; if (v >= 0) pn_n[q.unit] = -1 - v; }
      else if (errors) atomicAdd(&q.dst->errors, errors);
    }
    if (wave == 0) pn_stat_item(17, t0, (unsigned long long)((q.A1 - q.A0) + (q.B1 - q.B0)));
  }
  pn_stats_flush();
}
__global__ __launch_bounds__(64) void anim_postnuc_forced_strips_kernel(const RefDesc* __restrict__ refs, const UnitDesc* __restrict__ units,
                                                                        PnForcedReq* __restrict__ reqs, uint32_t* __restrict__ cursor,
                                                                        int32_t* __restrict__ pn_n, uint32_t* __restrict__ gscratch,
                                                                        const uint32_t* __restrict__ strips, const uint32_t* __restrict__ n_strips) {
  __shared__ uint32_t lds[3 * 4 * PN_LDS_CELLS];
  __shared__ uint32_t s_i;
  const int lane = threadIdx.x & 63;
  pn_stats_begin();
  const uint32_t n_items = *n_strips;
  for (;;) {
    __syncthreads();
    if (lane == 0) s_i = atomicAdd(cursor, 1u);
    __syncthreads();
    const uint32_t i = pn_uni(s_i);
    if (i >= n_items) break;
    const uint32_t slot = pn_uni(strips[i]);
    const PnForcedReq q = reqs[slot];
    const unsigned long long t0 = wall_clock64();
    const UnitDesc U = units[q.unit];
    const RefDesc Rd = refs[U.ref];
    int32_t err = 0, w_used = 0, w_next = 0;
    const int st = pn_forced_wave<true, true>(SeqView{Rd.codes, Rd.mask, Rd.len}, StrandView{SeqView{U.codes, U.mask, U.len}, U.strand}, lds,
                                              gscratch + (size_t)blockIdx.x * PN_GLOBAL_WORDS, q.A0, q.A1, q.B0, q.B1, q.w, err, w_used, w_next, 0u);
    if (lane == 0) {
      reqs[slot].w = w_used;
      if (st != 0) { const int32_t v = pn_n[q.unit]; if (v >= 0) pn_n[q.unit] = -1 - v; }
      else if (err) atomicAdd(&q.dst->errors, err);
    }
    pn_stat_item(17, t0, (unsigned long long)((q.A1 - q.A0) + (q.B1 - q.B0)));
  }
  pn_stats_flush();
}

constexpr int PN_SMALL = 59;
struct PnGapTask { uint32_t unit, slot; };

template <int C>
__global__ __launch_bounds__(64) void anim_postnuc_gaplane_kernel(const RefDesc* __restrict__ refs, const UnitDesc* __restrict__ units, ClusterOut O,
                                                                  const PnGapTask* __restrict__ tasks, const uint32_t* __restrict__ n_tasks,
                                                                  pgn::PnGap* __restrict__ gaps) {
  using namespace pgn;
  const uint32_t n = *n_tasks;
  for (uint32_t t0 = blockIdx.x * 64u; t0 < n; t0 += gridDim.x * 64u) {
    const uint32_t t = t0 + (threadIdx.x & 63);
    const bool live = t < n;
    const PnGapTask T = tasks[live ? t : 0];
    const UnitDesc U = units[T.unit];
    const RefDesc Rd = refs[U.ref];
    const size_t off = O.moff[T.unit];
    const Match a = O.cm[off + T.slot], b = O.cm[off + T.slot + 1];
    const int32_t A0 = a.r + a.len - 1, B0 = a.q + a.len - 1;
    const int32_t N = live ? b.r - A0 + 1 : 0, M = live ? b.q - B0 + 1 : 0;
    const StrandView Q{SeqView{U.codes, U.mask, U.len}, U.strand};
    uint64_t aw[2], bw[2]; uint32_t ak[2], bk[2];
    packed_window(Rd.codes, Rd.mask, Rd.len, A0, aw[0], ak[0]);
    packed_window(Rd.codes, Rd.mask, Rd.len, (int64_t)A0 + 32, aw[1], ak[1]);
    strand_window(Q, B0, bw[0], bk[0]);
    strand_window(Q, (int64_t)B0 + 32, bw[1], bk[1]);
    uint32_t X[C + 1], I[C + 1];
    X[0] = w_make(0, 0, ST_MATCH); I[0] = 0u;
#pragma unroll
    for (int j = 1; j <= C; ++j) {
// ... 379 lines not shown
```

### pyani_amd/csrc/pga_postnuc_diag.inc

```

__device__ __forceinline__ void strand_window(const StrandView& Q, int64_t p0, uint64_t& c, uint32_t& ok) {
  if (!Q.rc) { packed_window(Q.s.codes, Q.s.mask, (int32_t)Q.s.len, p0, c, ok); return; }
  uint64_t w; uint32_t k;
  packed_window(Q.s.codes, Q.s.mask, (int32_t)Q.s.len, Q.s.len - 32 - p0, w, k);
  const uint32_t lo = rev_fields2((uint32_t)(w >> 32)), hi = rev_fields2((uint32_t)w);
  c = ~(((uint64_t)hi << 32) | lo);
  ok = __brev(k);
}
__device__ __forceinline__ void rev_window32(uint64_t& c, uint32_t& ok) {
  const uint32_t lo = rev_fields2((uint32_t)(c >> 32)), hi = rev_fields2((uint32_t)c);
  c = ((uint64_t)hi << 32) | lo;
  ok = __brev(ok);
}
struct PnRawWin { uint32_t c0, c1, c2, m0, m1; };
__device__ __forceinline__ PnRawWin packed_window_load(const uint32_t* __restrict__ codes, const uint32_t* __restrict__ mask, int32_t len, int64_t p0) {
  const bool out = p0 >= len || p0 + 32 <= 0;
  const int64_t q0 = out ? 0 : (p0 < 0 ? 0 : p0);
  const int32_t w = (int32_t)(q0 >> 4), lastw = len > 0 ? (len - 1) >> 4 : 0;
  const int32_t mw = (int32_t)(q0 >> 5), lastm = len > 0 ? (len - 1) >> 5 : 0;
  PnRawWin r;
  r.c0 = codes[w]; r.c1 = codes[w + 1 <= lastw ? w + 1 : lastw]; r.c2 = codes[w + 2 <= lastw ? w + 2 : lastw];
  r.m0 = mask[mw]; r.m1 = mask[mw + 1 <= lastm ? mw + 1 : lastm];
  return r;
}
// ... 81 lines not shown
      C.update_best(gk, gw);
    }
    const uint32_t thr = C.trim_threshold();
    uint64_t m[DPL / 2], all = 0ull;
#pragma unroll
    for (int t = 0; t < DPL / 2; ++t) { m[t] = __ballot(T.X[PAR + 2 * t] >= thr); all |= m[t]; }
    any = all != 0ull;
    if (any) {
      const int l0 = (int)__builtin_ctzll(all), l1 = 63 - (int)__builtin_clzll(all);
      int s0 = pn_bit_select2<PAR + DPL - 4, PAR + DPL - 2>(m[DPL / 2 - 2], l0), s1 = pn_bit_select2<PAR + 2, PAR>(m[1], l1);
#pragma unroll
      for (int t = DPL / 2 - 3; t >= 0; --t) s0 = pn_bit_select_t<PAR>(t, m[t], l0, s0);
#pragma unroll
      for (int t = 2; t < DPL / 2; ++t) s1 = pn_bit_select_t<PAR>(t, m[t], l1, s1);
      gmin = (uint32_t)(DPL * l0 + s0); gmax = (uint32_t)(DPL * l1 + s1);
    }
  }
  C.template end_step<FORCED, !FORCED && PAR == 1>(any, gmin, gmax);
}

template <int DPL, int PAR, bool FORCED, bool INFO>
__device__ __forceinline__ bool pn_diag_advance(pgd::DiagRegs<DPL>& T, pgd::DiagCtl& C, const SeqView& R, const StrandView& Q, int32_t Astart,
                                                int32_t Bstart, int lane, uint32_t& stat_moves, const pgd::DiagRelabel& relmask,
                                                PnRawWin& na, PnRawWin& nb, bool& have_next) {
  constexpr int32_t W = 64 * DPL;
  if (!C.template begin_step_go<FORCED>()) return false;
  if (__builtin_expect(((C.lo - 2) | (W - 3 - C.hi)) < 0, 0)) {
    const int32_t n = C.template window_check<DPL>();
    if (n == INT32_MIN) { C.Dend = INT32_MIN; return false; }
#pragma unroll
    for (int s = 0; s < DPL; ++s) {
      const int src = lane + n;
      const uint32_t x = (uint32_t)__shfl((int)T.X[s], src & 63, 64), d = (uint32_t)__shfl((int)T.D[s], src & 63, 64), i = (uint32_t)__shfl((int)T.I[s], src & 63, 64);
      const bool ok = src >= 0 && src < 64;
      T.X[s] = ok ? x : 0u; T.D[s] = ok ? d : 0u; T.I[s] = ok ? i : 0u;
    }
    C.template window_move<DPL>(n);
    ++stat_moves;
    have_next = false;
  }
  if (C.Dct == C.next_refill) { pn_diag_refill<DPL, PAR, 32 * DPL, !FORCED>(T, R, Q, C, Astart, Bstart, lane, na, nb, have_next); C.next_refill = C.Dct + 32; }
  C.template note_cells<INFO>();
  pn_diag_step<DPL, PAR, FORCED>(T, C, lane, relmask);
  return true;
}

template <int DPL, bool FORCED, bool INFO>
__device__ bool pn_align_diag_run(const SeqView& R_, const StrandView& Q_, int32_t Astart_, int32_t& Aend, int32_t Bstart_, int32_t& Bend,
                                  unsigned m_o_, int32_t band_w_, int32_t& errors, int32_t& score, bool& reached, PnRunInfo* info,
                                  int kstat) {
  using namespace pgd;
  constexpr int32_t HALF = 32 * DPL;
  const int lane = threadIdx.x & 63;
  const SeqView R = pn_uni(R_);
  const StrandView Q = pn_uni(Q_);
  const int32_t Astart = pn_uni(Astart_), Bstart = pn_uni(Bstart_), Aend0 = pn_uni(Aend), Bend0 = pn_uni(Bend);
  const unsigned m_o = pn_uni((uint32_t)m_o_);
  const bool fwd = m_o & DIRECTION_BIT;
  DiagCtl C;
  C.template init<DPL>(fwd ? Aend0 - Astart + 1 : Astart - Aend0 + 1, fwd ? Bend0 - Bstart + 1 : Bstart - Bend0 + 1, m_o, pn_uni(band_w_));
  DiagRegs<DPL> T;
#pragma unroll
  for (int s = 0; s < DPL; ++s) { T.X[s] = 0u; T.D[s] = 0u; T.I[s] = 0u; T.mw[s] = 0u; }
  if (lane == HALF / DPL) T.X[0] = FORCED ? w_make(0, 0, ST_MATCH) : (NORM_BIAS << SCORE_SHIFT) | ST_MATCH;
  uint32_t stat_moves = 0;
  DiagRelabel relmask;
  asm volatile("v_mov_b32 %0, 0xfffe7fff" : "=v"(relmask.mask));
  asm volatile("v_mov_b32 %0, 0x8000" : "=v"(relmask.st_insert));
  asm volatile("v_mov_b32 %0, 0x10000" : "=v"(relmask.st_match));
  PnRawWin na{0u, 0u, 0u, 0u, 0u}, nb{0u, 0u, 0u, 0u, 0u};
  bool have_next = false;
  for (;;) {
    if (!pn_diag_advance<DPL, 1, FORCED, INFO>(T, C, R, Q, Astart, Bstart, lane, stat_moves, relmask, na, nb, have_next)) break;
    if (!pn_diag_advance<DPL, 0, FORCED, INFO>(T, C, R, Q, Astart, Bstart, lane, stat_moves, relmask, na, nb, have_next)) break;
  }
  {
    const uint32_t keep = (uint32_t)(C.ga ^ C.gb ^ C.lo ^ C.hi ^ C.c1g ^ C.c2g ^ C.next_refill) ^ C.high_fw ^ C.thr_w;
    asm volatile("" ::"s"(keep));
  }
  if (C.Dend == INT32_MIN) { pn_stat(10, 1); return false; }
  const unsigned long long cells = C.cells_total();
  if (info) { info->cells = cells; info->wmax = C.wmax; }
  pn_stat(0, 1); pn_stat(1, (unsigned long long)C.steps()); pn_stat(2, cells); pn_stat(9, stat_moves);
  if (kstat >= 0) pn_kstat(kstat, 1ull, (unsigned long long)C.steps(), cells);
  uint32_t corner = 0u, fin_w = C.high_w;
  bool rch = false;
  int32_t FinishK = 0;
  if (C.template finish1<DPL>(rch, corner, FinishK)) {
    const int src = __builtin_amdgcn_readfirstlane((int)(corner / DPL));
    const uint32_t cs = corner % DPL;
    uint32_t v = 0u;
#pragma unroll
    for (int s = 0; s < DPL; ++s) if (cs == (uint32_t)s) v = T.X[s];
    fin_w = (uint32_t)__builtin_amdgcn_readlane((int)v, src);
  }
  reached = rch;
  C.template finish2<!FORCED>(fin_w, FinishK, Astart, Bstart, Aend, Bend, errors, score);
  return true;
}
template <int DPL>
__device__ __forceinline__ bool pn_align_diag(const SeqView& R, const StrandView& Q, int32_t Astart, int32_t& Aend, int32_t Bstart, int32_t& Bend,
                                              unsigned m_o, int32_t band_w, int32_t& errors, int32_t& score, bool& reached, PnRunInfo* info = nullptr,
                                              int kstat = -1) {
  if (pn_uni((uint32_t)m_o) & pgn::FORCED_BIT) return pn_align_diag_run<DPL, true, false>(R, Q, Astart, Aend, Bstart, Bend, m_o, band_w, errors, score, reached, info, kstat);
  if constexpr (DPL < 4) return false;
  else {
    if (info) return pn_align_diag_run<DPL, false, true>(R, Q, Astart, Aend, Bstart, Bend, m_o, band_w, errors, score, reached, info, kstat);
    return pn_align_diag_run<DPL, false, false>(R, Q, Astart, Aend, Bstart, Bend, m_o, band_w, errors, score, reached, info, kstat);
  }
}

template <int NW, int DPL>
__device__ bool pn_forced_diag_group(const SeqView& R_, const StrandView& Q_, int32_t A0_, int32_t A1_, int32_t B0_, int32_t B1_, int32_t band_w_,
                                     uint32_t* xch, int32_t& errors, int32_t& score, int kstat) {
  using namespace pgd;
  constexpr int DPLE = DPL * NW, W = 64 * DPLE, HALF = W / 2;
  const int lane = threadIdx.x & 63, wave = __builtin_amdgcn_readfirstlane((int)(threadIdx.x >> 6)), glane = 64 * wave + lane;
  const SeqView R = pn_uni(R_);
  const StrandView Q = pn_uni(Q_);
  const int32_t A0 = pn_uni(A0_), A1 = pn_uni(A1_), B0 = pn_uni(B0_), B1 = pn_uni(B1_), band_w = pn_uni(band_w_);
  DiagCtl C;
  C.template init<DPLE>(A1 - A0 + 1, B1 - B0 + 1, FORCED_FORWARD_ALIGN, band_w);
  {
    const int32_t klo = band_w >= 0 ? C.kming - HALF : -C.N, khi = band_w >= 0 ? C.kmaxg - HALF : C.M;
    C.window_shift(2 * ((klo + khi) / 4));
    if (klo - C.shiftk + HALF < 2 || khi - C.shiftk + HALF > W - 3) return false;
  }
  DiagRegs<DPL> T;
#pragma unroll
  for (int s = 0; s < DPL; ++s) { T.X[s] = 0u; T.D[s] = 0u; T.I[s] = 0u; T.mw[s] = 0u; }
  {
    const int32_t g = 0 - C.shiftk + HALF;
#pragma unroll
    for (int s = 0; s < DPL; ++s) if (glane == g / DPL && (g % DPL) == s) T.X[s] = w_make(0, 0, ST_MATCH);
  }
  DiagRelabel rel;
  asm volatile("v_mov_b32 %0, 0xfffe7fff" : "=v"(rel.mask));
  asm volatile("v_mov_b32 %0, 0x8000" : "=v"(rel.st_insert));
  asm volatile("v_mov_b32 %0, 0x10000" : "=v"(rel.st_match));
  PnRawWin na{0u, 0u, 0u, 0u, 0u}, nb{0u, 0u, 0u, 0u, 0u};
  bool have_next = false;
  int why = 0, buf = 0;
  while (!why) {
    why = C.template begin_step<true>();
    if (!why && (C.lo < 2 || C.hi > W - 3)) why = 3;
    if (why) break;
    const int par = C.Dct & 1;
    if (C.Dct == C.next_refill) {
      if (par) pn_diag_refill<DPL, 1, HALF>(T, R, Q, C, A0, B0, glane, na, nb, have_next); else pn_diag_refill<DPL, 0, HALF>(T, R, Q, C, A0, B0, glane, na, nb, have_next);
      C.next_refill = C.Dct + 32;
    }
    C.template note_cells<false>();
    uint32_t* mine = xch + (buf * NW + wave) * 4;
    const uint32_t edge = par == 0 ? diag_lane_edge<DPL, 0>(T) : diag_lane_edge<DPL, 1>(T);
    if (par == 0) { if (lane == 63) mine[0] = edge; }
    else { if (lane == 0) mine[2] = edge; }
    __syncthreads();
    uint32_t key, keyw;
    if (par == 0) {
      uint32_t nbM = dpp_from_below0(edge);
      if (lane == 0 && wave > 0) nbM = xch[(buf * NW + wave - 1) * 4];
      diag_lane_step<DPL, 0, false>(T, nbM, (uint32_t)(DPL * glane), (uint32_t)C.lo, (uint32_t)(C.hi - C.lo), rel, key, keyw);
    } else {
      uint32_t nbM = dpp_from_above0(edge);
      if (lane == 63 && wave + 1 < NW) nbM = xch[(buf * NW + wave + 1) * 4 + 2];
      diag_lane_step<DPL, 1, false>(T, nbM, (uint32_t)(DPL * glane), (uint32_t)C.lo, (uint32_t)(C.hi - C.lo), rel, key, keyw);
    }
    C.template end_step<true>(false, 0u, 0u);
    buf ^= 1;
  }
  if (why == 3) return false;
  const unsigned long long cells = C.cells_total();
  if (wave == 0) { pn_stat(0, 1); pn_stat(1, (unsigned long long)C.steps()); pn_stat(2, cells); if (kstat >= 0) pn_kstat(kstat, 1ull, (unsigned long long)C.steps(), cells); }
  uint32_t corner = 0u, fin_w = C.high_w;
  bool rch = false;
  int32_t FinishK = 0;
  uint32_t* res = xch + 2 * NW * 4;
  __syncthreads();
  if (C.template finish1<DPLE>(rch, corner, FinishK)) {
#pragma unroll
    for (int s = 0; s < DPL; ++s) if (glane == (int)(corner / DPL) && (corner % DPL) == (uint32_t)s) res[0] = T.X[s];
    __syncthreads();
    fin_w = res[0];
  }
  if (!rch) return false;
  int32_t a = A1, b = B1;
  C.finish2(fin_w, FinishK, A0, B0, a, b, errors, score);
  __syncthreads();
  return true;
}
```

### pyani_amd/engine.py

```python
import ctypes
from pathlib import Path
from typing import Iterable, List, Optional, Sequence, Tuple

import numpy as np

from . import _lib


def _ptr(a: Optional[np.ndarray]):
    return None if a is None else a.ctypes.data


class Engine:
    def __init__(self, device: int = 0):
        self.lib = _lib.load()
        h = ctypes.c_void_p()
        rc = self.lib.pg_create(ctypes.byref(h), device)
        if rc == _lib.PG_E_NODEVICE:
            raise _lib.PyaniGpuError(rc, "no HIP device visible: pyani_amd needs an MI355X (there is no CPU fallback)")
        if rc != 0:
            raise _lib.PyaniGpuError(rc, "pg_create failed")
        self._h = h
        self.device = device

# ... 69 lines not shown

    @staticmethod
    def _ids(ids) -> np.ndarray:
        return np.ascontiguousarray(list(ids), dtype=np.int32)

    def tetra_counts(self, ids) -> Tuple[np.ndarray, np.ndarray, np.ndarray]:
        a = self._ids(ids)
        n = len(a)
        c2, c3, c4 = (np.zeros((n, k), dtype=np.uint64) for k in (16, 64, 256))
        self._check(self.lib.pg_tetra_counts(self._h, a.ctypes.data, n, c2.ctypes.data, c3.ctypes.data, c4.ctypes.data))
        return c2, c3, c4

    def tetra_zscores_from_counts(self, c2, c3, c4) -> Tuple[np.ndarray, np.ndarray]:
        c2, c3, c4 = (np.ascontiguousarray(x, dtype=np.uint64).reshape(-1, k) for x, k in ((c2, 16), (c3, 64), (c4, 256)))
        n = c4.shape[0]
        z = np.zeros((n, 256), dtype=np.float64)
        present = np.zeros((n, 256), dtype=np.uint8)
        self._check(self.lib.pg_tetra_zscores(self._h, c2.ctypes.data, c3.ctypes.data, c4.ctypes.data, n, z.ctypes.data,
                                              present.ctypes.data))
        return z, present

    def tetra_corr(self, z: np.ndarray, present: np.ndarray) -> np.ndarray:
        z = np.ascontiguousarray(z, dtype=np.float64).reshape(-1, 256)
        present = np.ascontiguousarray(present, dtype=np.uint8).reshape(-1, 256)
        n = z.shape[0]
        out = np.zeros((n, n), dtype=np.float64)
        self._check(self.lib.pg_tetra_corr(self._h, z.ctypes.data, present.ctypes.data, n, out.ctypes.data))
        return out

    def tetra_matrix(self, ids, want_corr: bool = True) -> Tuple[np.ndarray, np.ndarray, Optional[np.ndarray]]:
        a = self._ids(ids)
        n = len(a)
        z = np.zeros((n, 256), dtype=np.float64)
        present = np.zeros((n, 256), dtype=np.uint8)
        corr = np.zeros((n, n), dtype=np.float64) if want_corr else None
        self._check(self.lib.pg_tetra_matrix(self._h, a.ctypes.data, n, z.ctypes.data, present.ctypes.data, _ptr(corr)))
        return z, present, corr

    def tetra_matrix_enqueue(self, ids_array: np.ndarray, fetch_z: bool = True):
        self._check(self.lib.pg_tetra_matrix_enqueue(self._h, ids_array.ctypes.data, len(ids_array), int(fetch_z)))

    def tetra_matrix_fetch(self, n: int) -> Tuple[np.ndarray, np.ndarray, np.ndarray]:
        z = np.zeros((n, 256), dtype=np.float64)
        present = np.zeros((n, 256), dtype=np.uint8)
        corr = np.zeros((n, n), dtype=np.float64)
        self._check(self.lib.pg_tetra_matrix_fetch(self._h, n, z.ctypes.data, present.ctypes.data, corr.ctypes.data))
        return z, present, corr

    def tetra_zscores_dev(self, ids, d_z_ptr: int, d_present_ptr: int):
        a = self._ids(ids)
        self._check(self.lib.pg_tetra_zscores_dev(self._h, a.ctypes.data, len(a), d_z_ptr, d_present_ptr))

    def tetra_corr_rows_dev(self, d_z_ptr: int, d_present_ptr: int, n: int, row0: int, nrows: int, d_out_ptr: int):
        self._check(self.lib.pg_tetra_corr_rows_dev(self._h, d_z_ptr, d_present_ptr, n, row0, nrows, d_out_ptr))

    ANIM_DTYPE = np.dtype([("ref_aln_len", "<i8"), ("qry_aln_len", "<i8"), ("sim_errors", "<i8"), ("n_alignments", "<i8"),
                           ("identity", "<f8"), ("status", "<i4"), ("reserved", "<i4")])

    def anim_pairs(self, ref_ids, qry_ids, filter_1to1: bool = True, maxmatch: bool = False) -> np.ndarray:
        r, q = self._ids(ref_ids), self._ids(qry_ids)
        if len(r) != len(q):
            raise ValueError("ref_ids and qry_ids must have the same length")
        out = np.zeros(len(r), dtype=self.ANIM_DTYPE)
        self._check(self.lib.pg_anim_pairs(self._h, r.ctypes.data, q.ctypes.data, len(r), int(maxmatch), int(filter_1to1),
                                           out.ctypes.data))
        return out

    def anim_pairs_enqueue(self, ref_ids, qry_ids, filter_1to1: bool = True, maxmatch: bool = False):
        r, q = self._ids(ref_ids), self._ids(qry_ids)
        if len(r) != len(q):
            raise ValueError("ref_ids and qry_ids must have the same length")
        t = ctypes.c_uint64(0)
        self._check(self.lib.pg_anim_pairs_enqueue(self._h, r.ctypes.data, q.ctypes.data, len(r), int(maxmatch), int(filter_1to1), ctypes.byref(t)))
        return (int(t.value), len(r))

    def anim_pairs_fetch(self, ticket) -> np.ndarray:
        tid, n = ticket
        out = np.zeros(n, dtype=self.ANIM_DTYPE)
        self._check(self.lib.pg_anim_pairs_fetch(self._h, ctypes.c_uint64(tid), out.ctypes.data, n))
        return out

    def anim_set_workers(self, workers: int = 2) -> None:
        self._check(self.lib.pg_anim_set_workers(self._h, int(workers)))

    def anim_counters(self, reset: bool = False) -> np.ndarray:
        out = np.zeros(64, dtype=np.uint64)
        self._check(self.lib.pg_anim_counters(self._h, out.ctypes.data, int(bool(reset))))
        return out

    def anim_set_batch_budget(self, max_pairs: int, max_matches: int) -> None:
        self._check(self.lib.pg_anim_set_batch_budget(self._h, int(max_pairs), int(max_matches)))

    ALN_DTYPE = np.dtype([("ref_rec", "<i4"), ("qry_rec", "<i4"), ("rs", "<i4"), ("re", "<i4"), ("qs", "<i4"), ("qe", "<i4"),
                          ("errors", "<i4"), ("kept", "<i4")])

    def anim_pair_alignments(self, ref_id: int, qry_id: int) -> np.ndarray:
        n = ctypes.c_uint32(0)
        out = np.zeros(4096, dtype=self.ALN_DTYPE)
        self._check(self.lib.pg_anim_pair_alignments(self._h, int(ref_id), int(qry_id), out.ctypes.data, len(out), ctypes.byref(n)))
        if n.value > len(out):
            out = np.zeros(n.value, dtype=self.ALN_DTYPE)
            self._check(self.lib.pg_anim_pair_alignments(self._h, int(ref_id), int(qry_id), out.ctypes.data, len(out), ctypes.byref(n)))
        return out[:n.value].copy()

    def anim_alignments_batch(self, ref_ids, qry_ids, maxmatch: bool = False, with_indels: bool = False):
        r = np.ascontiguousarray(list(ref_ids), dtype=np.int32)
        q = np.ascontiguousarray(list(qry_ids), dtype=np.int32)
        if len(r) != len(q):
            raise ValueError("ref_ids and qry_ids must have the same length")
        offsets = np.zeros(len(r) + 1, dtype=np.uint64)
        n_ind = ctypes.c_uint64(0)
        self._check(self.lib.pg_anim_alignments_batch(self._h, r.ctypes.data, q.ctypes.data, len(r), int(bool(maxmatch)), int(bool(with_indels)),
                                                      offsets.ctypes.data, ctypes.byref(n_ind)))
        recs = np.zeros(int(offsets[-1]), dtype=self.ALN_DTYPE)
        ioff = np.zeros(len(recs) + 1, dtype=np.uint64) if with_indels else None
        ind = np.zeros(int(n_ind.value), dtype=np.int64) if with_indels else None
        self._check(self.lib.pg_anim_alignments_read(self._h, recs.ctypes.data if len(recs) else None, ioff.ctypes.data if with_indels else None,
                                                     ind.ctypes.data if with_indels and len(ind) else None))
        return offsets, recs, ioff, ind

    def anim_reduce(self, pairs, apply_filter: bool = False) -> np.ndarray:
        offsets = np.zeros(len(pairs) + 1, dtype=np.uint64)
        for k, recs in enumerate(pairs):
            offsets[k + 1] = offsets[k] + len(recs)
        flat = np.array([r for recs in pairs for r in recs], dtype=np.int32).reshape(-1, 7)
        cols = [np.ascontiguousarray(flat[:, c]) for c in range(7)]
        out = np.zeros(len(pairs), dtype=self.ANIM_DTYPE)
        self._check(self.lib.pg_anim_reduce(self._h, len(pairs), offsets.ctypes.data, *(c.ctypes.data for c in cols),
                                            int(apply_filter), out.ctypes.data))
        return out

    def anib_reduce(self, pairs):
        n = len(pairs)
        offsets = np.zeros(n + 1, dtype=np.uint64)
        nfr = np.zeros(max(n, 1), dtype=np.uint32)
        for k, (nf, rows) in enumerate(pairs):
            offsets[k + 1] = offsets[k] + len(rows)
            nfr[k] = nf
        flat = [r for _, rows in pairs for r in rows]
        ints = np.array([r[:5] for r in flat], dtype=np.int32).reshape(-1, 5)
        cols = [np.ascontiguousarray(ints[:, c]) for c in range(5)]
        pid = np.ascontiguousarray([r[5] for r in flat], dtype=np.float64)
        aln, err, out = np.zeros(n, dtype=np.int64), np.zeros(n, dtype=np.int64), np.zeros(n, dtype=np.float64)
        self._check(self.lib.pg_anib_reduce(self._h, n, offsets.ctypes.data, nfr.ctypes.data, cols[0].ctypes.data,
                                            cols[1].ctypes.data, cols[2].ctypes.data, cols[3].ctypes.data, cols[4].ctypes.data,
                                            pid.ctypes.data, aln.ctypes.data, err.ctypes.data, out.ctypes.data))
        return aln, err, out

    ANIB_DTYPE = np.dtype([("aln_length", "<i8"), ("sim_errors", "<i8"), ("pid", "<f8"), ("n_frags", "<i4"), ("n_kept", "<i4"),
                           ("status", "<i4"), ("reserved", "<i4")])
    ANIB_ROW_DTYPE = np.dtype([("frag", "<i4"), ("length", "<i4"), ("mismatch", "<i4"), ("gaps", "<i4"), ("nident", "<i4"),
                               ("qlen", "<i4"), ("qstart", "<i4"), ("qend", "<i4"), ("sstart", "<i4"), ("send", "<i4"), ("srec", "<i4"),
                               ("score", "<i4")])

    def anib_pairs(self, qry_ids, sbj_ids, fragsize: int = 1020) -> np.ndarray:
        q, s = self._ids(qry_ids), self._ids(sbj_ids)
        if len(q) != len(s):
            raise ValueError("qry_ids and sbj_ids must have the same length")
        out = np.zeros(len(q), dtype=self.ANIB_DTYPE)
        self._check(self.lib.pg_anib_pairs(self._h, q.ctypes.data, s.ctypes.data, len(q), int(fragsize), out.ctypes.data))
        return out

    def anib_pair_rows(self, qry_id: int, sbj_id: int, fragsize: int = 1020) -> np.ndarray:
        n = ctypes.c_uint32(0)
        nfr, _ = self.genome_length(qry_id)
        out = np.zeros(4 * (nfr // max(1, fragsize) + 4096), dtype=self.ANIB_ROW_DTYPE)
# ... 44 lines not shown
```

Measured before the change: 65390.

## Exchange ghost lanes per block in multi-wave forced diagonal DP instead of every step

The multi-wave group kernel for wide forced alignments now overlaps waves by two ghost lanes (62 live lanes per wave) and swaps full lane state through LDS once every DPL anti-diagonals, replacing the per-step edge exchange and __syncthreads. This is meant to cut block-wide barriers and LDS traffic in the inner DP loop, at the cost of redundant ghost-lane work and slightly narrower windows. The change also adds finer DPL forms (10, 20, 28), lowers the group span cap to match the new lane geometry, adds a host emulator, and adds atomics-based histogram instrumentation that runs unconditionally on the device.

```diff
diff --git a/include/pyani_gpu.h b/include/pyani_gpu.h
--- a/include/pyani_gpu.h
+++ b/include/pyani_gpu.h
@@ -73,6 +73,8 @@
 
 int pg_anim_counters(pg_ctx* ctx, uint64_t* out, int reset);
 
+int pg_anim_forced_hist(pg_ctx* ctx, uint64_t* out, int reset);
+
 int pg_anim_set_batch_budget(pg_ctx* ctx, uint32_t max_pairs, uint64_t max_matches);
 
 typedef struct {
diff --git a/pyani_amd/_lib.py b/pyani_amd/_lib.py
--- a/pyani_amd/_lib.py
+++ b/pyani_amd/_lib.py
@@ -54,6 +54,7 @@
     "pg_anim_set_workers": (_int, [_vp, _int]),
     "pg_anim_set_extender": (_int, [_vp, _int]),
     "pg_anim_counters": (_int, [_vp, _vp, _int]),
+    "pg_anim_forced_hist": (_int, [_vp, _vp, _int]),
     "pg_anim_pair_alignments": (_int, [_vp, _i32, _i32, _vp, _u32, _P(_u32)]),
     "pg_anim_alignments_batch": (_int, [_vp, _vp, _vp, _u64, _int, _int, _vp, _P(_u64)]),
     "pg_anim_alignments_read": (_int, [_vp, _vp, _vp, _vp]),
diff --git a/pyani_amd/csrc/pg_anim.hip b/pyani_amd/csrc/pg_anim.hip
--- a/pyani_amd/csrc/pg_anim.hip
+++ b/pyani_amd/csrc/pg_anim.hip
@@ -176,6 +176,14 @@
 }
 
 void pg_anim_set_sink(PgAlnSink* sink) { tls_sink = sink; }
+int pg_anim_forced_hist_read(pg_ctx* ctx, uint64_t* out, int reset) {
+  PG_HIP(ctx, hipDeviceSynchronize());
+  unsigned long long a[PN_FH_SIZE], z[PN_FH_SIZE] = {0};
+  PG_HIP(ctx, hipMemcpyFromSymbol(a, HIP_SYMBOL(g_pn_fhist), sizeof(a)));
+  for (int i = 0; i < PN_FH_SIZE; ++i) out[i] = a[i];
+  if (reset) PG_HIP(ctx, hipMemcpyToSymbol(HIP_SYMBOL(g_pn_fhist), z, sizeof(z)));
+  return PG_OK;
+}
 int pg_anim_counters_read(pg_ctx* ctx, uint64_t* out, int reset) {
   PG_HIP(ctx, hipDeviceSynchronize());
   unsigned long long a[32], b[32], z[32] = {0};
@@ -891,7 +899,7 @@
                          A->pn_wide + req_cap, A->pn_cursor + 14, win_max);
       hipLaunchKernelGGL(anim_postnuc_forced_huge_kernel, dim3((uint32_t)ctx->num_cu * 2u), dim3(64 * PN_HUGE_WAVES), 0, cur_stream(ctx), A->refs_d,
                          A->units_d, A->pn_reqs, A->pn_cursor + 15, A->pn_n, A->pn_wide + req_cap, A->pn_cursor + 14, A->pn_wide + 2 * req_cap,
-                         A->pn_cursor + 16, group_max);
+                         A->pn_cursor + 16, group_max, (uint32_t)ctx->anim_pn_group_min_dpl);
       hipLaunchKernelGGL(anim_postnuc_forced_strips_kernel, dim3(pn_waves), dim3(64), 0, cur_stream(ctx), A->refs_d, A->units_d, A->pn_reqs,
                          A->pn_cursor + 17, A->pn_n, A->pn_gscratch, A->pn_wide + 2 * req_cap, A->pn_cursor + 16);
     }
@@ -913,6 +921,19 @@
         const char* kn[8] = {"gaps", "forward", "backward-ahead", "walks", "forced narrow", "forced 512-1024", "forced 2048", "forced group 8192"};
         for (int k = 0; k < 8; ++k)
           fprintf(stderr, "[pn-stats] diagonal engine in %-16s: %llu calls, %llu anti-diagonals, %llu cells\n", kn[k], ks[4 * k], ks[4 * k + 1], ks[4 * k + 2]);
+        for (int k = 4; k < 8; ++k)
+          fprintf(stderr, "[pn-stats] %-16s: %llu slot-steps, live-slot fraction %.4f\n", kn[k], ks[4 * k + 3], ks[4 * k + 3] ? (double)ks[4 * k + 2] / (double)ks[4 * k + 3] : 0.0);
+        unsigned long long fh[PN_FH_SIZE], fz[PN_FH_SIZE] = {0};
+        PG_HIP(ctx, hipMemcpyFromSymbol(fh, HIP_SYMBOL(g_pn_fhist), sizeof(fh)));
+        PG_HIP(ctx, hipMemcpyToSymbol(HIP_SYMBOL(g_pn_fhist), fz, sizeof(fz)));
+        for (int g = 0; g < 2; ++g) {
+          fprintf(stderr, "[pn-stats] forced passes by window form (%s kernel, diagonals:passes):", g ? "group" : "wide");
+          for (int d = 1; d <= 16; ++d) if (fh[(g ? PN_FH_GROUP : PN_FH_WIDE) + d]) fprintf(stderr, " %d:%llu", (g ? 250 : 64) * 2 * d, fh[(g ? PN_FH_GROUP : PN_FH_WIDE) + d]);
+          fprintf(stderr, "\n");
+        }
+        fprintf(stderr, "[pn-stats] forced span histogram of the wide + group kernels (span from:passes/anti-diagonals):");
+        for (int b = 0; b < 128; ++b) if (fh[PN_FH_PASSES + b]) fprintf(stderr, " %d:%llu/%llu", 64 * b, fh[PN_FH_PASSES + b], fh[PN_FH_STEPS + b]);
+        fprintf(stderr, "\n");
         fprintf(stderr, "[pn-stats] walk kernel scans: shadow test %.1f ms over %llu rows of 64 alignments, reverse-target search %.1f ms in %llu calls (summed over waves)\n",
                 ks[3] / 1e5, ks[7], ks[11] / 1e5, ks[15]);
         fprintf(stderr, "[pn-stats] run-ahead results the walk took: forward %llu of %llu computed (%.4f), backward %llu found ready of %llu searches run ahead; %llu searches left to the walk itself\n",
diff --git a/pyani_amd/csrc/pg_api.cpp b/pyani_amd/csrc/pg_api.cpp
--- a/pyani_amd/csrc/pg_api.cpp
+++ b/pyani_amd/csrc/pg_api.cpp
@@ -317,6 +317,7 @@
   if (const char* g = pg_dev_env("PYANI_ANIM_BWD_AHEAD")) ctx->anim_bwd_ahead = atoi(g) != 0;
   if (const char* g = pg_dev_env("PYANI_PN_WINDOW_MAX")) ctx->anim_pn_window_max = atoi(g);
   if (const char* g = pg_dev_env("PYANI_PN_GROUP_MAX")) ctx->anim_pn_group_max = atoi(g);
+  if (const char* g = pg_dev_env("PYANI_PN_GROUP_MIN_DPL")) ctx->anim_pn_group_min_dpl = atoi(g);
   if (const char* g = pg_dev_env("PYANI_ANIM_GAP_LANES")) ctx->anim_gap_lanes = atoi(g) != 0;
   if (const char* w = pg_dev_env("PYANI_ANIM_WORKERS")) {
     ctx->anim_workers = atoi(w);
@@ -741,6 +742,12 @@
   if (!ctx || workers < 1 || workers > pg_ctx::MAX_WORKERS) return pg_fail(ctx, PG_E_ARG, "workers must be 1 ... 4");
   ctx->anim_workers = workers;
   return PG_OK;
+}
+
+int pg_anim_forced_hist(pg_ctx* ctx, uint64_t* out, int reset) {
+  if (!ctx || !out) return pg_fail(ctx, PG_E_ARG, "bad argument");
+  PG_HIP(ctx, hipSetDevice(ctx->device));
+  return pg_anim_forced_hist_read(ctx, out, reset);
 }
 
 int pg_anim_counters(pg_ctx* ctx, uint64_t* out, int reset) {
diff --git a/pyani_amd/csrc/pg_internal.h b/pyani_amd/csrc/pg_internal.h
--- a/pyani_amd/csrc/pg_internal.h
+++ b/pyani_amd/csrc/pg_internal.h
@@ -82,7 +82,8 @@
   std::mutex anim_mu, err_mu, prof_mu;
   int anib_word_tier = 1;
   int anim_pn_window_max = 2048;
-  int anim_pn_group_max = 8184;
+  int anim_pn_group_max = 7992;
+  int anim_pn_group_min_dpl = 0;
   int anim_gap_lanes = 1;
   int anim_bwd_ahead = 1;
   int anim_workers = 2;
@@ -148,6 +149,7 @@
   std::vector<std::vector<int64_t>> indels;
 };
 int pg_anim_counters_read(pg_ctx* ctx, uint64_t* out , int reset);
+int pg_anim_forced_hist_read(pg_ctx* ctx, uint64_t* out , int reset);
 void pg_anim_set_sink(PgAlnSink* sink);
 void pg_anim_drop_lists(pg_ctx* ctx);
 void pg_sketch_drop(pg_ctx* ctx);
diff --git a/pyani_amd/csrc/pg_nucmer_diag.h b/pyani_amd/csrc/pg_nucmer_diag.h
--- a/pyani_amd/csrc/pg_nucmer_diag.h
+++ b/pyani_amd/csrc/pg_nucmer_diag.h
@@ -1,5 +1,8 @@
 #pragma once
 #include <stdint.h>
+#if !defined(__HIP_DEVICE_COMPILE__)
+#include <vector>
+#endif
 #include "pg_nucmer_core.h"
 
 namespace pgd {
@@ -127,9 +130,8 @@
   uint32_t span_sum;
   int32_t wmax;
   int32_t next_refill;
-  template <int DPL>
+  template <int DPL, int32_t HALF = 32 * DPL>
   PG_HD void init(int32_t N_, int32_t M_, unsigned m_o, int32_t band_w) {
-    constexpr int32_t HALF = 32 * DPL;
     N = N_; M = M_; NM = N_ + M_;
     fwd = m_o & DIRECTION_BIT; forced = m_o & FORCED_BIT; optimal = m_o & OPTIMAL_BIT; banded = band_w >= 0;
     kming = (M - N < 0 ? M - N : 0) - band_w + HALF; kmaxg = (M - N > 0 ? M - N : 0) + band_w + HALF;
@@ -202,9 +204,8 @@
     ++Dct; ++c1g; --c2g;
     if (NORM_EVEN) { high_fw -= (uint32_t)GOOD_SCORE << SCORE_SHIFT; thr_w -= (uint32_t)GOOD_SCORE << SCORE_SHIFT; }
   }
-  template <int DPL>
+  template <int DPL, int32_t HALF = 32 * DPL>
   PG_HD bool finish1(bool& reached, uint32_t& corner_slot, int32_t& FinishK) {
-    constexpr int32_t HALF = 32 * DPL;
     reached = false;
     const int32_t last = Dct - 1;
     corner_slot = 0u;
@@ -315,6 +316,109 @@
 };
 #endif
 
+#if !defined(__HIP_DEVICE_COMPILE__)
+template <int NW, int DPL, typename RefT, typename QryT, int BLOCK = DPL>
+struct DiagGroupEmu {
+  static constexpr int GL = 62 * NW + 2, W = GL * DPL, HALF = W / 2;
+  static_assert(BLOCK % 2 == 0 && HALF % 2 == 0, "whole (odd, even) pairs; slot and diagonal parities agree");
+  const RefT& R;
+  const QryT& Q;
+  long cells = 0, calls = 0, exchanges = 0;
+  DiagRegs<DPL> T[NW][64];
+  std::vector<uint64_t>* trace = nullptr;
+  DiagGroupEmu(const RefT& R_, const QryT& Q_) : R(R_), Q(Q_) {}
+  static int glane(int w, int l) { return 62 * w + l; }
+  template <int PAR>
+  void refill(const DiagCtl& C, int32_t A0, int32_t B0) {
+    for (int w = 0; w < NW; ++w)
+      for (int l = 0; l < 64; ++l) {
+        const int32_t k0 = DPL * glane(w, l) - HALF + C.shiftk;
+        int32_t ia0, jb0;
+        diag_refill_origin<DPL, PAR>(C.Dct, k0, ia0, jb0);
+        uint64_t ca = 0, cb = 0; uint32_t oka = 0, okb = 0;
+        for (int f = 0; f < 32; ++f) {
+          const int64_t pa = (int64_t)A0 + (ia0 + f) - 1, pb = (int64_t)B0 + (jb0 + f) - 1;
+          if (R.clean(pa)) { ca |= (uint64_t)R.base(pa) << (2 * f); oka |= 1u << f; }
+          if (Q.clean(pb)) { cb |= (uint64_t)Q.base(pb) << (2 * f); okb |= 1u << f; }
+        }
+        diag_lane_refill<DPL, PAR, false, false>(T[w][l], ca, oka, cb, okb);
+      }
+  }
+  template <int PAR>
+  void step(DiagCtl& C) {
+    uint32_t key, keyw;
+    for (int w = 0; w < NW; ++w) {
+      uint32_t nbM[64];
+      for (int l = 0; l < 64; ++l) {
+        if (PAR == 0) nbM[l] = l > 0 ? diag_lane_edge<DPL, PAR>(T[w][l - 1]) : 0u;
+        else nbM[l] = l < 63 ? diag_lane_edge<DPL, PAR>(T[w][l + 1]) : 0u;
+      }
+      for (int l = 0; l < 64; ++l)
+        diag_lane_step<DPL, PAR, false>(T[w][l], nbM[l], (uint32_t)(DPL * glane(w, l)), (uint32_t)C.lo, (uint32_t)(C.hi - C.lo),
+                                        DiagRelabel{~W_STATE, ST_INSERT, ST_MATCH}, key, keyw);
+    }
+    C.template end_step<true>(false, 0u, 0u);
+  }
+  void exchange() {
+    for (int w = 0; w < NW; ++w)
+      for (int s = 0; s < DPL; ++s) {
+        if (w > 0) { T[w][0].X[s] = T[w - 1][62].X[s]; T[w][0].D[s] = T[w - 1][62].D[s]; T[w][0].I[s] = T[w - 1][62].I[s]; }
+        if (w + 1 < NW) { T[w][63].X[s] = T[w + 1][1].X[s]; T[w][63].D[s] = T[w + 1][1].D[s]; T[w][63].I[s] = T[w + 1][1].I[s]; }
+      }
+    ++exchanges;
+  }
+  template <int PAR>
+  bool advance(DiagCtl& C, int32_t A0, int32_t B0) {
+    if (!C.template begin_step_go<true>()) return false;
+    if (C.lo < 2 || C.hi > W - 3) { C.Dend = INT32_MIN; return false; }
+    if (C.Dct == C.next_refill) { refill<PAR>(C, A0, B0); C.next_refill = C.Dct + 32; }
+    C.template note_cells<false>();
+    step<PAR>(C);
+    if (trace) {
+      uint64_t h = 1469598103934665603ull;
+      for (int w = 0; w < NW; ++w)
+        for (int l = (w > 0 ? 1 : 0); l < (w + 1 < NW ? 63 : 64); ++l)
+          for (int s = 0; s < DPL; ++s)
+            for (uint32_t v : {T[w][l].X[s], T[w][l].D[s], T[w][l].I[s]}) h = (h ^ v) * 1099511628211ull;
+      trace->push_back(h);
+    }
+    return true;
+  }
+  bool run(int32_t A0, int32_t A1, int32_t B0, int32_t B1, int32_t band_w, int32_t& errors, int32_t& score) {
+    DiagCtl C;
+    C.template init<DPL, HALF>(A1 - A0 + 1, B1 - B0 + 1, FORCED_FORWARD_ALIGN, band_w);
+    const int32_t klo = band_w >= 0 ? C.kming - HALF : -C.N, khi = band_w >= 0 ? C.kmaxg - HALF : C.M;
+    C.window_shift(2 * ((klo + khi) / 4));
+    if (klo - C.shiftk + HALF < 2 || khi - C.shiftk + HALF > W - 3) return false;
+    for (int w = 0; w < NW; ++w)
+      for (int l = 0; l < 64; ++l)
+        for (int s = 0; s < DPL; ++s) { T[w][l].X[s] = 0u; T[w][l].D[s] = 0u; T[w][l].I[s] = 0u; T[w][l].mw[s] = 0u; }
+    const int32_t g = 0 - C.shiftk + HALF;
+    for (int w = 0; w < NW; ++w)
+      for (int l = 0; l < 64; ++l) if (glane(w, l) == g / DPL) T[w][l].X[g % DPL] = w_make(0, 0, ST_MATCH);
+    ++calls;
+    for (bool go = true; go;) {
+      for (int p = 0; p < BLOCK / 2 && go; ++p) go = advance<1>(C, A0, B0) && advance<0>(C, A0, B0);
+      if (go) exchange();
+    }
+    if (C.Dend == INT32_MIN) return false;
+    cells += (long)C.cells_total();
+    uint32_t corner = 0u, fin_w = C.high_w;
+    bool rch = false;
+    int32_t FinishK = 0;
+    if (C.template finish1<DPL, HALF>(rch, corner, FinishK)) {
+      const int gl = (int)(corner / DPL);
+      const int w = gl == 0 ? 0 : gl == GL - 1 ? NW - 1 : (gl - 1) / 62;
+      fin_w = T[w][gl - 62 * w].X[corner % DPL];
+    }
+    if (!rch) return false;
+    int32_t a = A1, b = B1;
+    C.finish2(fin_w, FinishK, A0, B0, a, b, errors, score);
+    return true;
+  }
+};
+#endif
+
 PG_HD bool diag_window_holds(int64_t span, int dpl) { return span <= 64 * (int64_t)dpl - 2 * (int64_t)dpl + 2; }
 #if !defined(__HIP_DEVICE_COMPILE__)
 template <typename RefT, typename QryT>
@@ -324,14 +428,18 @@
   DiagWaveEmu<4, RefT, QryT> e4;
   DiagWaveEmu<6, RefT, QryT> e6;
   DiagWaveEmu<8, RefT, QryT> e8;
+  DiagWaveEmu<10, RefT, QryT> e10;
   DiagWaveEmu<12, RefT, QryT> e12;
+  DiagWaveEmu<14, RefT, QryT> e14;
   DiagWaveEmu<16, RefT, QryT> e16;
+  DiagWaveEmu<20, RefT, QryT> e20;
   DiagWaveEmu<24, RefT, QryT> e24;
+  DiagWaveEmu<28, RefT, QryT> e28;
   DiagWaveEmu<32, RefT, QryT> e32;
   long fallbacks = 0;
   void (*fallback_log)(int32_t N, int32_t M, unsigned m_o, int32_t band_w) = nullptr;
   DiagWaveEngine(const RefT& R, const QryT& Q, Cell* d0, Cell* d1, Cell* d2, int32_t cap)
-      : slow{R, Q, d0, d1, d2, cap}, e2{R, Q}, e4{R, Q}, e6{R, Q}, e8{R, Q}, e12{R, Q}, e16{R, Q}, e24{R, Q}, e32{R, Q} {}
+      : slow{R, Q, d0, d1, d2, cap}, e2{R, Q}, e4{R, Q}, e6{R, Q}, e8{R, Q}, e10{R, Q}, e12{R, Q}, e14{R, Q}, e16{R, Q}, e20{R, Q}, e24{R, Q}, e28{R, Q}, e32{R, Q} {}
   bool gap_ready(int32_t, PnGap&) const { return false; }
   void piece(uint32_t, int32_t, int32_t, int32_t, int32_t, int32_t, int32_t, int32_t, unsigned) {}
   bool bwd_ready(int, PnBwd&) const { return false; }
@@ -355,7 +463,7 @@
     if (!(m_o & FORCED_BIT)) return 256;
     const int32_t df = N < M ? M - N : N - M;
     const int64_t span = band_w >= 0 ? (int64_t)df + 2 * (int64_t)band_w + 1 : (int64_t)N + M + 1;
-    for (int w : {128, 256, 384, 512, 768, 1024, 1536, 2048}) if (diag_window_holds(span + 5, w / 64)) return w;
+    for (int w : {128, 256, 384, 512, 640, 768, 896, 1024, 1280, 1536, 1792, 2048}) if (diag_window_holds(span + 5, w / 64)) return w;
     return 0;
   }
   bool run(int32_t Astart, int32_t& Aend, int32_t Bstart, int32_t& Bend, unsigned m_o, int32_t band_w, int32_t& errors, int32_t& score) {
@@ -368,9 +476,13 @@
       case 256: done = e4.run(Astart, a, Bstart, b, m_o, band_w, errors, score, reached); break;
       case 384: done = e6.run(Astart, a, Bstart, b, m_o, band_w, errors, score, reached); break;
       case 512: done = e8.run(Astart, a, Bstart, b, m_o, band_w, errors, score, reached); break;
+      case 640: done = e10.run(Astart, a, Bstart, b, m_o, band_w, errors, score, reached); break;
       case 768: done = e12.run(Astart, a, Bstart, b, m_o, band_w, errors, score, reached); break;
+      case 896: done = e14.run(Astart, a, Bstart, b, m_o, band_w, errors, score, reached); break;
       case 1024: done = e16.run(Astart, a, Bstart, b, m_o, band_w, errors, score, reached); break;
+      case 1280: done = e20.run(Astart, a, Bstart, b, m_o, band_w, errors, score, reached); break;
       case 1536: done = e24.run(Astart, a, Bstart, b, m_o, band_w, errors, score, reached); break;
+      case 1792: done = e28.run(Astart, a, Bstart, b, m_o, band_w, errors, score, reached); break;
       case 2048: done = e32.run(Astart, a, Bstart, b, m_o, band_w, errors, score, reached); break;
       default: break;
     }
diff --git a/pyani_amd/csrc/pga_postnuc.inc b/pyani_amd/csrc/pga_postnuc.inc
--- a/pyani_amd/csrc/pga_postnuc.inc
+++ b/pyani_amd/csrc/pga_postnuc.inc
@@ -22,6 +22,14 @@
 
 __device__ unsigned long long g_pn_stats[32];
 __device__ unsigned long long g_pn_kstats[32];
+constexpr int PN_FH_PASSES = 0, PN_FH_STEPS = 128, PN_FH_WIDE = 256, PN_FH_GROUP = 288, PN_FH_SIZE = 320;
+__device__ unsigned long long g_pn_fhist[PN_FH_SIZE];
+__device__ __forceinline__ void pn_fhist(int64_t span, int32_t steps, int form_at) {
+  if ((threadIdx.x & 63) == 0) {
+    const int b = span >= 64 * 127 ? 127 : (int)(span >> 6);
+    atomicAdd(&g_pn_fhist[PN_FH_PASSES + b], 1ull); atomicAdd(&g_pn_fhist[PN_FH_STEPS + b], (unsigned long long)steps); atomicAdd(&g_pn_fhist[form_at], 1ull);
+  }
+}
 __device__ __forceinline__ unsigned long long* pn_stats_lds() { __shared__ unsigned long long s_pn[64]; return s_pn; }
 __device__ __forceinline__ void pn_stats_begin() {
   unsigned long long* s = pn_stats_lds();
@@ -42,6 +50,9 @@
 __device__ __forceinline__ void pn_stat_max(int k, unsigned long long v) { if ((threadIdx.x & 63) == 0) atomicMax(&pn_stats_lds()[k], v); }
 __device__ __forceinline__ void pn_kstat(int k, unsigned long long calls, unsigned long long steps, unsigned long long cells) {
   if ((threadIdx.x & 63) == 0) { unsigned long long* s = pn_stats_lds() + 32 + 4 * k; atomicAdd(&s[0], calls); atomicAdd(&s[1], steps); atomicAdd(&s[2], cells); }
+}
+__device__ __forceinline__ void pn_kstat_slots(int k, unsigned long long slot_steps) {
+  if ((threadIdx.x & 63) == 0 && k >= 4) atomicAdd(&pn_stats_lds()[32 + 4 * k + 3], slot_steps);
 }
 __device__ __forceinline__ void pn_stat_item(int k, unsigned long long t0, unsigned long long size) {
   const unsigned long long t1 = wall_clock64(), sz = size < 0xFFFFFull ? size : 0xFFFFFull;
@@ -577,15 +588,17 @@
     if (!WIDE && (!pgd::diag_window_holds(span, 8) || win_max < 128u)) { w_next = w; return 1; }
     const unsigned long long t0 = wall_clock64();
     const int cls = span <= 256 ? 0 : span <= 512 ? 1 : span <= 2048 ? 2 : 3;
+    int form = 0;
 #define PN_TRY_DIAG(DPL_, KSTAT_) \
-    if (!done && 64u * DPL_ <= win_max && pgd::diag_window_holds(span, DPL_)) { a = A1; b = B1; done = pn_align_diag<DPL_>(R, Q, A0, a, B0, b, m_o, bw, errors, score, reached, nullptr, KSTAT_); }
+    if (!done && 64u * DPL_ <= win_max && pgd::diag_window_holds(span, DPL_)) { a = A1; b = B1; form = DPL_; done = pn_align_diag<DPL_>(R, Q, A0, a, B0, b, m_o, bw, errors, score, reached, nullptr, KSTAT_); }
     if (!WIDE) {
       PN_TRY_DIAG(2, 4) PN_TRY_DIAG(4, 4) PN_TRY_DIAG(6, 4) PN_TRY_DIAG(8, 4)
       if (!done) { w_next = w; return 1; }
     } else {
-      PN_TRY_DIAG(8, 5) PN_TRY_DIAG(12, 5) PN_TRY_DIAG(16, 5) PN_TRY_DIAG(24, 6) PN_TRY_DIAG(32, 6)
+      PN_TRY_DIAG(8, 5) PN_TRY_DIAG(10, 5) PN_TRY_DIAG(12, 5) PN_TRY_DIAG(14, 5) PN_TRY_DIAG(16, 5) PN_TRY_DIAG(20, 6) PN_TRY_DIAG(24, 6)
+      PN_TRY_DIAG(28, 6) PN_TRY_DIAG(32, 6)
 #undef PN_TRY_DIAG
-      if (done) {}
+      if (done) pn_fhist(span, N + M, PN_FH_WIDE + form / 2);
       else if (!STRIPS) { w_next = w; return 1; }
       else if ((size_t)(N + 1) * 8 <= PN_GLOBAL_WORDS) {
         done = true;
@@ -668,8 +681,8 @@
 __global__ __launch_bounds__(64 * PN_HUGE_WAVES) __attribute__((amdgpu_waves_per_eu(2, 2))) void anim_postnuc_forced_huge_kernel(
     const RefDesc* __restrict__ refs, const UnitDesc* __restrict__ units, PnForcedReq* __restrict__ reqs, uint32_t* __restrict__ cursor,
     int32_t* __restrict__ pn_n, const uint32_t* __restrict__ huge, const uint32_t* __restrict__ n_huge, uint32_t* __restrict__ strips,
-    uint32_t* __restrict__ n_strips, uint32_t group_max) {
-  __shared__ uint32_t xch[2 * PN_HUGE_WAVES * 4 + 4];
+    uint32_t* __restrict__ n_strips, uint32_t group_max, uint32_t group_min_dpl) {
+  __shared__ __attribute__((aligned(16))) uint32_t xch[2 * PN_HUGE_WAVES * 2 * 3 * 32 + 4];
   __shared__ uint32_t s_i;
   const int wave = (int)(threadIdx.x >> 6);
   pn_stats_begin();
@@ -698,10 +711,12 @@
       bool done = false;
       const unsigned long long t1 = wall_clock64();
       if (span <= (int64_t)group_max) {
-        if (span <= 64 * 12 * PN_HUGE_WAVES - 8) done = pn_forced_diag_group<PN_HUGE_WAVES, 12>(R, Q, A0, A1, B0, B1, bw, xch, errors, score, 7);
-        else if (span <= 64 * 16 * PN_HUGE_WAVES - 8) done = pn_forced_diag_group<PN_HUGE_WAVES, 16>(R, Q, A0, A1, B0, B1, bw, xch, errors, score, 7);
-        else if (span <= 64 * 24 * PN_HUGE_WAVES - 8) done = pn_forced_diag_group<PN_HUGE_WAVES, 24>(R, Q, A0, A1, B0, B1, bw, xch, errors, score, 7);
-        else if (span <= 64 * 32 * PN_HUGE_WAVES - 8) done = pn_forced_diag_group<PN_HUGE_WAVES, 32>(R, Q, A0, A1, B0, B1, bw, xch, errors, score, 7);
+        int form = 0;
+#define PN_TRY_GROUP(DPL_) \
+        if (!form && DPL_ >= group_min_dpl && span <= pn_group_lanes<PN_HUGE_WAVES>() * DPL_ - 8) { form = DPL_; done = pn_forced_diag_group<PN_HUGE_WAVES, DPL_>(R, Q, A0, A1, B0, B1, bw, xch, errors, score, 7); }
+        PN_TRY_GROUP(10) PN_TRY_GROUP(12) PN_TRY_GROUP(16) PN_TRY_GROUP(20) PN_TRY_GROUP(24) PN_TRY_GROUP(28) PN_TRY_GROUP(32)
+#undef PN_TRY_GROUP
+        if (done && wave == 0) pn_fhist(span, N + M, PN_FH_GROUP + form / 2);
       }
       if (!done) {
         if (threadIdx.x == 0) { reqs[slot].w = w; strips[atomicAdd(n_strips, 1u)] = slot; }
diff --git a/pyani_amd/csrc/pga_postnuc_diag.inc b/pyani_amd/csrc/pga_postnuc_diag.inc
--- a/pyani_amd/csrc/pga_postnuc_diag.inc
+++ b/pyani_amd/csrc/pga_postnuc_diag.inc
@@ -187,7 +187,7 @@
   const unsigned long long cells = C.cells_total();
   if (info) { info->cells = cells; info->wmax = C.wmax; }
   pn_stat(0, 1); pn_stat(1, (unsigned long long)C.steps()); pn_stat(2, cells); pn_stat(9, stat_moves);
-  if (kstat >= 0) pn_kstat(kstat, 1ull, (unsigned long long)C.steps(), cells);
+  if (kstat >= 0) { pn_kstat(kstat, 1ull, (unsigned long long)C.steps(), cells); pn_kstat_slots(kstat, (unsigned long long)C.steps() * HALF); }
   uint32_t corner = 0u, fin_w = C.high_w;
   bool rch = false;
   int32_t FinishK = 0;
@@ -215,17 +215,32 @@
   }
 }
 
+template <int DPL, int PAR, int HALF, int W>
+__device__ __forceinline__ bool pn_group_advance(pgd::DiagRegs<DPL>& T, pgd::DiagCtl& C, const SeqView& R, const StrandView& Q, int32_t A0,
+                                                 int32_t B0, int glane, const pgd::DiagRelabel& rel, PnRawWin& na, PnRawWin& nb, bool& have_next) {
+  if (!C.template begin_step_go<true>()) return false;
+  if (__builtin_expect(((C.lo - 2) | (W - 3 - C.hi)) < 0, 0)) { C.Dend = INT32_MIN; return false; }
+  if (C.Dct == C.next_refill) { pn_diag_refill<DPL, PAR, HALF>(T, R, Q, C, A0, B0, glane, na, nb, have_next); C.next_refill = C.Dct + 32; }
+  C.template note_cells<false>();
+  pn_diag_step<DPL, PAR, true>(T, C, glane, rel);
+  return true;
+}
+
+template <int NW>
+constexpr int pn_group_lanes() { return 62 * NW + 2; }
 template <int NW, int DPL>
 __device__ bool pn_forced_diag_group(const SeqView& R_, const StrandView& Q_, int32_t A0_, int32_t A1_, int32_t B0_, int32_t B1_, int32_t band_w_,
                                      uint32_t* xch, int32_t& errors, int32_t& score, int kstat) {
   using namespace pgd;
-  constexpr int DPLE = DPL * NW, W = 64 * DPLE, HALF = W / 2;
-  const int lane = threadIdx.x & 63, wave = __builtin_amdgcn_readfirstlane((int)(threadIdx.x >> 6)), glane = 64 * wave + lane;
+  constexpr int W = pn_group_lanes<NW>() * DPL, HALF = W / 2, XW = 3 * DPL;
+  static_assert(DPL % 2 == 0 && HALF % 2 == 0, "whole (odd, even) pairs per block; slot and diagonal parities agree");
+  const int lane = threadIdx.x & 63, wave = __builtin_amdgcn_readfirstlane((int)(threadIdx.x >> 6)), glane = 62 * wave + lane;
+  const bool ghost = (lane == 0 && wave > 0) || (lane == 63 && wave + 1 < NW);
   const SeqView R = pn_uni(R_);
   const StrandView Q = pn_uni(Q_);
   const int32_t A0 = pn_uni(A0_), A1 = pn_uni(A1_), B0 = pn_uni(B0_), B1 = pn_uni(B1_), band_w = pn_uni(band_w_);
   DiagCtl C;
-  C.template init<DPLE>(A1 - A0 + 1, B1 - B0 + 1, FORCED_FORWARD_ALIGN, band_w);
+  C.template init<DPL, HALF>(A1 - A0 + 1, B1 - B0 + 1, FORCED_FORWARD_ALIGN, band_w);
   {
     const int32_t klo = band_w >= 0 ? C.kming - HALF : -C.N, khi = band_w >= 0 ? C.kmaxg - HALF : C.M;
     C.window_shift(2 * ((klo + khi) / 4));
@@ -245,46 +260,40 @@
   asm volatile("v_mov_b32 %0, 0x10000" : "=v"(rel.st_match));
   PnRawWin na{0u, 0u, 0u, 0u, 0u}, nb{0u, 0u, 0u, 0u, 0u};
   bool have_next = false;
-  int why = 0, buf = 0;
-  while (!why) {
-    why = C.template begin_step<true>();
-    if (!why && (C.lo < 2 || C.hi > W - 3)) why = 3;
-    if (why) break;
-    const int par = C.Dct & 1;
-    if (C.Dct == C.next_refill) {
-      if (par) pn_diag_refill<DPL, 1, HALF>(T, R, Q, C, A0, B0, glane, na, nb, have_next); else pn_diag_refill<DPL, 0, HALF>(T, R, Q, C, A0, B0, glane, na, nb, have_next);
-      C.next_refill = C.Dct + 32;
-    }
-    C.template note_cells<false>();
-    uint32_t* mine = xch + (buf * NW + wave) * 4;
-    const uint32_t edge = par == 0 ? diag_lane_edge<DPL, 0>(T) : diag_lane_edge<DPL, 1>(T);
-    if (par == 0) { if (lane == 63) mine[0] = edge; }
-    else { if (lane == 0) mine[2] = edge; }
+  const bool sends = (lane == 1 && wave > 0) || (lane == 62 && wave + 1 < NW);
+  const int out_at = (wave * 2 + (lane == 62 ? 1 : 0)) * XW, in_at = ghost ? ((lane == 0 ? (wave - 1) * 2 + 1 : (wave + 1) * 2) * XW) : 0;
+  int buf = 0;
+  for (bool go = true; go;) {
+#pragma unroll 1
+    for (int p = 0; p < DPL / 2 && go; ++p) {
+      go = pn_group_advance<DPL, 1, HALF, W>(T, C, R, Q, A0, B0, glane, rel, na, nb, have_next) &&
+           pn_group_advance<DPL, 0, HALF, W>(T, C, R, Q, A0, B0, glane, rel, na, nb, have_next);
+    }
+    if (!go) break;
+    uint32_t* x = xch + buf * (NW * 2 * XW);
+    if (sends) {
+#pragma unroll
+      for (int s = 0; s < DPL; ++s) { x[out_at + s] = T.X[s]; x[out_at + DPL + s] = T.D[s]; x[out_at + 2 * DPL + s] = T.I[s]; }
+    }
     __syncthreads();
-    uint32_t key, keyw;
-    if (par == 0) {
-      uint32_t nbM = dpp_from_below0(edge);
-      if (lane == 0 && wave > 0) nbM = xch[(buf * NW + wave - 1) * 4];
-      diag_lane_step<DPL, 0, false>(T, nbM, (uint32_t)(DPL * glane), (uint32_t)C.lo, (uint32_t)(C.hi - C.lo), rel, key, keyw);
-    } else {
-      uint32_t nbM = dpp_from_above0(edge);
-      if (lane == 63 && wave + 1 < NW) nbM = xch[(buf * NW + wave + 1) * 4 + 2];
-      diag_lane_step<DPL, 1, false>(T, nbM, (uint32_t)(DPL * glane), (uint32_t)C.lo, (uint32_t)(C.hi - C.lo), rel, key, keyw);
-    }
-    C.template end_step<true>(false, 0u, 0u);
+#pragma unroll
+    for (int s = 0; s < DPL; ++s) {
+      const uint32_t vx = x[in_at + s], vd = x[in_at + DPL + s], vi = x[in_at + 2 * DPL + s];
+      T.X[s] = ghost ? vx : T.X[s]; T.D[s] = ghost ? vd : T.D[s]; T.I[s] = ghost ? vi : T.I[s];
+    }
     buf ^= 1;
   }
-  if (why == 3) return false;
+  if (C.Dend == INT32_MIN) return false;
   const unsigned long long cells = C.cells_total();
-  if (wave == 0) { pn_stat(0, 1); pn_stat(1, (unsigned long long)C.steps()); pn_stat(2, cells); if (kstat >= 0) pn_kstat(kstat, 1ull, (unsigned long long)C.steps(), cells); }
+  if (wave == 0) { pn_stat(0, 1); pn_stat(1, (unsigned long long)C.steps()); pn_stat(2, cells); if (kstat >= 0) { pn_kstat(kstat, 1ull, (unsigned long long)C.steps(), cells); pn_kstat_slots(kstat, (unsigned long long)C.steps() * HALF); } }
   uint32_t corner = 0u, fin_w = C.high_w;
   bool rch = false;
   int32_t FinishK = 0;
-  uint32_t* res = xch + 2 * NW * 4;
+  uint32_t* res = xch + 2 * NW * 2 * XW;
   __syncthreads();
-  if (C.template finish1<DPLE>(rch, corner, FinishK)) {
-#pragma unroll
-    for (int s = 0; s < DPL; ++s) if (glane == (int)(corner / DPL) && (corner % DPL) == (uint32_t)s) res[0] = T.X[s];
+  if (C.template finish1<DPL, HALF>(rch, corner, FinishK)) {
+#pragma unroll
+    for (int s = 0; s < DPL; ++s) if (!ghost && glane == (int)(corner / DPL) && (corner % DPL) == (uint32_t)s) res[0] = T.X[s];
     __syncthreads();
     fin_w = res[0];
   }
diff --git a/pyani_amd/engine.py b/pyani_amd/engine.py
--- a/pyani_amd/engine.py
+++ b/pyani_amd/engine.py
@@ -175,6 +175,11 @@
 
     def anim_set_workers(self, workers: int = 2) -> None:
         self._check(self.lib.pg_anim_set_workers(self._h, int(workers)))
+
+    def anim_forced_hist(self, reset: bool = False) -> np.ndarray:
+        out = np.zeros(320, dtype=np.uint64)
+        self._check(self.lib.pg_anim_forced_hist(self._h, out.ctypes.data, int(bool(reset))))
+        return out
 
     def anim_counters(self, reset: bool = False) -> np.ndarray:
         out = np.zeros(64, dtype=np.uint64)
```

Result: faster. 67820, median of 6 (+3.7%).
